# speedinghzl/DSRG

Hardware: NVIDIA H100
Metric: images/s, SRG + DenseCRF pass at 321x321x21 (higher is better)
Workload: dtype f32

## Files before the change

dsrg_b200/csrc/api.cu:

```cuda
#include <math.h>
#include <stdarg.h>
#include <stdlib.h>
#include <string.h>

#include <map>
#include <mutex>
#include <utility>
#include <new>
#include <vector>

#include "common.cuh"

namespace dsrg {

static thread_local char g_err[512] = "";

void set_error(const char *fmt, ...) {
    va_list ap;
    va_start(ap, fmt);
    vsnprintf(g_err, sizeof(g_err), fmt, ap);
    va_end(ap);
}

int device_alloc(Engine *e, void **p, size_t bytes) {
    if (bytes == 0) bytes = 16;
    cudaError_t err = cudaMalloc(p, bytes);
    if (err != cudaSuccess) {
        set_error("cudaMalloc(%zu bytes) failed: %s", bytes, cudaGetErrorString(err));
        *p = nullptr;
        return DSRG_E_NOMEM;
    }
    e->bytes += bytes;
    return DSRG_OK;
}

static void lattice_scales(Lattice &L) {
    const float inv_std_dev = (float)(sqrt(2.0 / 3.0) * (L.d + 1));
    for (int i = 0; i < L.d; i++)
        L.scale[i] = (float)(1.0 / sqrt((double)((i + 2) * (i + 1))) * (double)inv_std_dev);
}

static bool key_range_ok(const Lattice &L, int W, int H) {
    double fmax[5] = {(W - 1) / (double)L.sigma[0], (H - 1) / (double)L.sigma[1], 0, 0, 0};
    for (int i = 2; i < L.d; i++) fmax[i] = 255.0 / (double)L.sigma[i];
    double sum = 0, big = 0;
    for (int i = 0; i < L.d; i++) {
        double cf = fabs(fmax[i]) * L.scale[i];
        sum += cf;
        if ((i + 1) * cf > big) big = (i + 1) * cf;
    }
    const double bound = sum + big + 3.0 * (L.d + 1) + 2;
    const int bits = (L.d == 2) ? 16 : 12;
    return bound < (double)((1 << (bits - 1)) - 1) && isfinite(bound);
}

static void lattice_shape(Engine *e, Lattice &L) {
    L.N = e->N;
    L.P = (4 - (e->N % 4)) % 4;
    L.capv = (L.N + L.P) * (L.d + 1);
    L.cap = 2 * L.capv;
    L.rows_cap = (long long)e->maxB * (L.capv + 1);
    L.nbr_stride = L.shared ? (long long)L.capv + 1 : L.rows_cap;
}

static void engine_shape(Engine *e, int H, int W) {
    e->H = H;
    e->W = W;
    e->N = H * W;
    e->tiles_x = (W + kTileW - 1) / kTileW;
    e->tile_w = (W + e->tiles_x - 1) / e->tiles_x;
    e->tiles_y = (H + kTileH - 1) / kTileH;
    e->ntiles = e->tiles_x * e->tiles_y;
    lattice_shape(e, e->sp);
    lattice_shape(e, e->bi);
    e->sp_valid = false;
}

static int lattice_alloc(Engine *e, Lattice &L, int d, int shared) {
    L.d = d;
    L.shared = shared;
    L.nimg = shared ? 1 : e->maxB;
    lattice_shape(e, L);
    const size_t n = (size_t)L.nimg;
    int rc = 0;
    rc |= dalloc(e, &L.off, n * (d + 1) * L.N);
    rc |= dalloc(e, &L.bary, n * (d + 1) * L.N);
    rc |= dalloc(e, &L.norm, n * L.N);
    rc |= dalloc(e, &L.hkeys, n * L.cap);
    rc |= dalloc(e, &L.hval, n * L.cap);
    rc |= dalloc(e, &L.vslot, n * L.capv);
    rc |= dalloc(e, &L.vcount, n);
    rc |= dalloc(e, &L.aslot, n * L.capv);
    rc |= dalloc(e, &L.vkey, n * L.capv);
    const long long rn_words = renum_words(e->ntiles, d + 1);
    rc |= dalloc(e, &L.rn_words, n * rn_words);
    rc |= dalloc(e, &L.rn_chunk, n * (rn_words / kRenumChunk));
    rc |= dalloc(e, &L.rowbase, (size_t)e->maxB + 1);
    rc |= dalloc(e, &L.nbr, (size_t)(d + 1) * L.nbr_stride);
    L.maxloc = (d == 2) ? kMaxLocSp : kMaxLocHy;
    const size_t nt = n * e->ntiles;
    rc |= dalloc(e, &L.tl_nloc, nt);
    rc |= dalloc(e, &L.tl_hy, nt);
    L.entcap = (kTileThreads * (d + 1) + L.maxloc + 7) & ~7;
    rc |= dalloc(e, &L.tl_hdr, nt * L.maxloc);
    rc |= dalloc(e, &L.tl_pack, nt * L.entcap);
    rc |= dalloc(e, &L.tl_loc, n * (d + 1) * L.N);
    rc |= dalloc(e, &L.wn, n * (d + 1) * L.N);
    if (rc) return DSRG_E_NOMEM;
    if (cudaMemset(L.hkeys, 0xFF, sizeof(uint64_t) * n * L.cap) != cudaSuccess) return DSRG_E_CUDA;
    if (cudaMemset(L.tl_hy, 0, nt) != cudaSuccess) return DSRG_E_CUDA;
    if (cudaMemset(L.hval, 0xFF, sizeof(int32_t) * n * L.cap) != cudaSuccess) return DSRG_E_CUDA;
    if (cudaMemset(L.vkey, 0x7F, sizeof(int32_t) * n * L.capv) != cudaSuccess) return DSRG_E_CUDA;
    return DSRG_OK;
}

static void lattice_free(Lattice &L) {
    cudaFree(L.off);
    cudaFree(L.bary);
    cudaFree(L.norm);
    cudaFree(L.hkeys);
    cudaFree(L.hval);
    cudaFree(L.vslot);
    cudaFree(L.vcount);
    cudaFree(L.aslot);
    cudaFree(L.vkey);
    cudaFree(L.rn_words);
    cudaFree(L.rn_chunk);
    cudaFree(L.rowbase);
    cudaFree(L.nbr);
    cudaFree(L.tl_nloc);
    cudaFree(L.tl_hy);
    cudaFree(L.tl_hdr);
    cudaFree(L.tl_pack);
    cudaFree(L.tl_loc);
    cudaFree(L.wn);
}

int check_device_flag(Engine *e, cudaStream_t s) {
    int flag = 0;
    DSRG_CUDA_TRY(cudaMemcpyAsync(&flag, e->dev_err, sizeof(int), cudaMemcpyDeviceToHost, s));
    DSRG_CUDA_TRY(cudaStreamSynchronize(s));
    if (flag != 0) {
        cudaMemsetAsync(e->dev_err, 0, sizeof(int), s);
        set_error("lattice coordinates exceed the packed-key range (sigma too small for this image size)");
        return flag;
    }
    return DSRG_OK;
}

static int prepare_lattices(Engine *e, int B, const uint8_t *image, const dsrg_crf_params &p,
                            cudaStream_t s) {
    if (!(p.theta_gamma_x > 0 && p.theta_gamma_y > 0 && p.theta_alpha_x > 0 && p.theta_alpha_y > 0 &&
          p.theta_beta_r > 0 && p.theta_beta_g > 0 && p.theta_beta_b > 0) || p.n_iters < 0) {
        set_error("CRF parameters must be positive");
        return DSRG_E_INVALID;
    }
    if (!e->sp_valid || e->sp.sigma[0] != p.theta_gamma_x || e->sp.sigma[1] != p.theta_gamma_y) {
        e->sp.sigma[0] = p.theta_gamma_x;
        e->sp.sigma[1] = p.theta_gamma_y;
        if (!key_range_ok(e->sp, e->W, e->H)) {
            set_error("spatial sigma (%g,%g) too small for %dx%d: lattice keys exceed 16 bits",
                      p.theta_gamma_x, p.theta_gamma_y, e->W, e->H);
            return DSRG_E_KEYRANGE;
        }
        int rc = lattice_build(e, e->sp, B, nullptr, s);
        if (rc) return rc;
        e->sp_valid = true;
    }
    e->bi.sigma[0] = p.theta_alpha_x;
    e->bi.sigma[1] = p.theta_alpha_y;
    e->bi.sigma[2] = p.theta_beta_r;
    e->bi.sigma[3] = p.theta_beta_g;
    e->bi.sigma[4] = p.theta_beta_b;
    if (!key_range_ok(e->bi, e->W, e->H)) {
        set_error("bilateral sigmas too small for %dx%d: lattice keys exceed the 12-bit packed range",
                  e->W, e->H);
        return DSRG_E_KEYRANGE;
    }
    return lattice_build(e, e->bi, B, image, s);
}

int check_batch(Engine *e, int B) {
    if (!e) {
        set_error("engine is NULL");
        return DSRG_E_INVALID;
    }
    if (B < 1 || B > e->maxB) {
        set_error("batch %d outside [1, %d]", B, e->maxB);
        return DSRG_E_INVALID;
    }
    int cur = -1;
    if (cudaGetDevice(&cur) != cudaSuccess || cur != e->device) DSRG_CUDA_TRY(cudaSetDevice(e->device));
    return DSRG_OK;
}

static bool spatial_ready(const Engine *e, const dsrg_crf_params *p) {
    return p && e->sp_valid && e->sp.sigma[0] == p->theta_gamma_x && e->sp.sigma[1] == p->theta_gamma_y;
}

static int crf_pass_done(Engine *e, int B, int rc) {
    if (rc == DSRG_OK) {
        e->Qcur = e->Q0;
        e->last_crf_B = B;
    } else {
        e->last_crf_B = 0;
    }
    return rc;
}

static GraphKey pass_key(const Engine *e, int entry, int B, const dsrg_crf_params *p) {
    GraphKey k;
    k.add(entry).add(B).add(e->H).add(e->W);
    if (p) k.add(*p);
    return k;
}

static int crf_core(Engine *e, int B, const float *unary, int layout, bool clamp, float *unary_rw,
                    const uint8_t *image, const dsrg_crf_params *p, cudaStream_t s) {
    if (layout != DSRG_LAYOUT_NHWC && layout != DSRG_LAYOUT_NCHW) {
        set_error("bad layout %d", layout);
        return DSRG_E_INVALID;
    }
    int rc = prepare_lattices(e, B, image, *p, s);
    if (rc) return rc;
    return meanfield_run(e, B, unary, layout, clamp, unary_rw, *p, s);
}

int crf_core_batch_for_post(Engine *e, int B, const float *unary_hwc, const uint8_t *images,
                            const dsrg_crf_params *p, cudaStream_t s) {
    return crf_core(e, B, unary_hwc, DSRG_LAYOUT_NHWC, false, nullptr, images, p, s);
}

bool post_pass_needs_spatial(const Engine *e, const dsrg_crf_params *p) { return !spatial_ready(e, p); }
void post_pass_done(Engine *e, const dsrg_crf_params *p, int B, int rc) {
    if (rc == DSRG_OK && p) {
        e->sp.sigma[0] = p->theta_gamma_x;
        e->sp.sigma[1] = p->theta_gamma_y;
        e->sp_valid = true;
    }
    crf_pass_done(e, B, rc);
}

int ensure_staging(Engine *e) {
    if (e->st_unary) return DSRG_OK;
    const size_t n = (size_t)e->maxB * e->M * e->Ncap;
    int rc = 0;
    rc |= dalloc(e, &e->st_unary, n);
    rc |= dalloc(e, &e->st_out, n);
    rc |= dalloc(e, &e->st_cues, n);
    rc |= dalloc(e, &e->st_labels, (size_t)e->maxB * e->M);
    rc |= dalloc(e, &e->st_image, (size_t)e->maxB * e->Ncap * 3);
    rc |= dalloc(e, &e->st_lmap, (size_t)e->maxB * e->Ncap);
    rc |= dalloc(e, &e->st_sel, (size_t)e->M);
    return rc ? DSRG_E_NOMEM : DSRG_OK;
}

int grow_staging(Engine *e, void **buf, size_t *cap_bytes, size_t bytes) {
    if (bytes <= *cap_bytes) return DSRG_OK;
    cudaFree(*buf);
    *buf = nullptr;
    *cap_bytes = 0;
    if (int rc = device_alloc(e, buf, bytes)) return rc;
    *cap_bytes = bytes;
    return DSRG_OK;
}

static int no_engine() {
    set_error("engine is NULL");
    return DSRG_E_INVALID;
}

static int last_crf_held(const Engine *e, int B) {
    if (e->last_crf_B == B) return DSRG_OK;
    set_error("no mean-field result for a batch of %d is held by this engine (last: %d)", B, e->last_crf_B);
    return DSRG_E_STATE;
}

static bool layout_ok(int layout) { return layout == DSRG_LAYOUT_NHWC || layout == DSRG_LAYOUT_NCHW; }

}

using namespace dsrg;

extern "C" {

int dsrg_version(void) { return 109; }

const char *dsrg_last_error(void) { return g_err; }

int dsrg_device_count(void) {
    int n = 0;
    if (cudaGetDeviceCount(&n) != cudaSuccess) {
        cudaGetLastError();
        return 0;
    }
    return n;
}

int dsrg_current_device(void) {
    if (const char *ev = getenv("DSRG_B200_DEVICE")) return atoi(ev);
    int dev = -1;
    if (cudaGetDevice(&dev) != cudaSuccess) {
        cudaGetLastError();
        return -1;
    }
    return dev;
}

void *dsrg_host_alloc(size_t bytes) {
    void *p = nullptr;
    if (numa_host_alloc(&p, bytes ? bytes : 16, dsrg_current_device()) != cudaSuccess) {
        set_error("cudaHostAlloc(%zu) failed", bytes);
        cudaGetLastError();
        return nullptr;
    }
    return p;
}

void dsrg_host_free(void *p) {
    if (p) cudaFreeHost(p);
}

int dsrg_host_register(void *p, size_t bytes) {
    if (!p || !bytes) return DSRG_E_INVALID;
    if (cudaHostRegister(p, bytes, cudaHostRegisterDefault) != cudaSuccess) {
        cudaGetLastError();
        set_error("cudaHostRegister(%zu bytes) failed", bytes);
        return DSRG_E_CUDA;
    }
    return DSRG_OK;
}

int dsrg_host_unregister(void *p) {
    if (!p) return DSRG_E_INVALID;
    if (cudaHostUnregister(p) != cudaSuccess) {
        cudaGetLastError();
        return DSRG_E_CUDA;
    }
    return DSRG_OK;
}

void dsrg_crf_params_default(dsrg_crf_params *p, float scale_factor, float color_factor, int maxiter) {
    p->w1 = 10.0f;
    p->theta_alpha_x = p->theta_alpha_y = (float)(80.0 / (double)scale_factor);
    p->theta_beta_r = p->theta_beta_g = p->theta_beta_b = color_factor;
    p->w2 = 3.0f;
    p->theta_gamma_x = p->theta_gamma_y = (float)(3.0 / (double)scale_factor);
    p->n_iters = maxiter;
}

dsrg_engine *dsrg_engine_create(int device, int max_batch, int H, int W, int M) {
    if (max_batch < 1 || H < 1 || W < 1 || M < 1 || M > DSRG_MAX_LABELS_WIDE ||
        (long long)H * W > (1ll << 24)) {
        set_error("bad engine shape (max_batch=%d H=%d W=%d M=%d; M <= %d)", max_batch, H, W, M,
                  DSRG_MAX_LABELS_WIDE);
        return nullptr;
    }
    int ndev = 0;
    if (device < 0) device = dsrg_current_device();
    if (cudaGetDeviceCount(&ndev) != cudaSuccess || device < 0 || device >= ndev) {
        cudaGetLastError();
        set_error("no usable CUDA device %d (visible devices: %d): this library has no CPU fallback",
                  device, ndev);
        return nullptr;
    }
    cudaDeviceProp prop;
    Engine probe;
    probe.device = device;
    DeviceScope dev_scope(&probe);
    if (cudaGetDeviceProperties(&prop, device) != cudaSuccess) {
        set_error("cannot select device %d", device);
        return nullptr;
    }
    if (prop.major != 9 || prop.minor != 0) {
        set_error("device %d is sm_%d%d; this build contains sm_90a code only", device, prop.major,
                  prop.minor);
        return nullptr;
    }
    Engine *e = new (std::nothrow) Engine();
    if (!e) return nullptr;
    e->device = device;
    if (numa_wanted()) {
        e->numa_node = numa_node_of_device(device);
        numa_bind_thread(e->numa_node);
    }
    e->maxB = max_batch;
    e->M = M;
    e->MP = (M + 3) / 4 * 4;
    e->sm_count = prop.multiProcessorCount;
    e->sp.d = 2;
    e->sp.shared = 1;
    e->bi.d = 5;
    e->Hcap = H;
    e->Wcap = W;
    e->Ncap = H * W;
    engine_shape(e, H, W);
    int rc = 0;
    rc |= lattice_alloc(e, e->sp, 2, 1);
    rc |= lattice_alloc(e, e->bi, 5, 0);
    lattice_scales(e->sp);
    lattice_scales(e->bi);
    const size_t n = (size_t)max_batch * M * e->N;
    rc |= dalloc(e, &e->U, n);
    rc |= dalloc(e, &e->Q0, n);
    rc |= dalloc(e, &e->spA, (size_t)e->sp.rows_cap * e->MP);
    rc |= dalloc(e, &e->spB, (size_t)e->sp.rows_cap * e->MP);
    rc |= dalloc(e, &e->spC, (size_t)e->sp.rows_cap * e->MP);
    rc |= dalloc(e, &e->biC, (size_t)e->bi.rows_cap * e->MP);
    rc |= dalloc(e, &e->biA, (size_t)e->bi.rows_cap * e->MP);
    rc |= dalloc(e, &e->biB, (size_t)e->bi.rows_cap * e->MP);
    rc |= dalloc(e, &e->nvA, (size_t)e->bi.rows_cap);
    rc |= dalloc(e, &e->nvB, (size_t)e->bi.rows_cap);
    const size_t bn = (size_t)max_batch * e->N;
    rc |= dalloc(e, &e->lmap, bn);
    rc |= dalloc(e, &e->lflag, bn);
    rc |= dalloc(e, &e->parent, bn);
    rc |= dalloc(e, &e->hc, bn);
    rc |= dalloc(e, &e->loss_acc, (size_t)max_batch * 4);
    e->sec_wcap = e->Ncap < DSRG_GWRP_MAX_PLANE ? e->Ncap : DSRG_GWRP_MAX_PLANE;
    rc |= dalloc(e, &e->sec_rec, (size_t)max_batch * M);
    rc |= dalloc(e, &e->sec_img, (size_t)max_batch * 3);
    rc |= dalloc(e, &e->sec_part, (size_t)max_batch * kSecPlainChunks);
    rc |= dalloc(e, &e->sec_w, (size_t)2 * e->sec_wcap);
    rc |= dalloc(e, &e->dev_err, 1);
    rc |= dalloc(e, &e->hy_list, (size_t)max_batch * e->ntiles);
    rc |= dalloc(e, &e->hy_count, 1);
    if (!rc && cudaMemset(e->hy_count, 0, sizeof(int)) != cudaSuccess) rc = DSRG_E_CUDA;
    if (!rc && cudaMemset(e->dev_err, 0, sizeof(int)) != cudaSuccess) rc = DSRG_E_CUDA;
    if (!rc && cudaStreamCreateWithFlags(&e->own_stream, cudaStreamNonBlocking) != cudaSuccess) rc = DSRG_E_CUDA;
    if (!rc && cudaStreamCreateWithFlags(&e->in_stream, cudaStreamNonBlocking) != cudaSuccess) rc = DSRG_E_CUDA;
    if (!rc && cudaEventCreateWithFlags(&e->order_event, cudaEventDisableTiming) != cudaSuccess) rc = DSRG_E_CUDA;
    if (const char *ev = getenv("DSRG_B200_WIRE")) e->wire_compress = atoi(ev) != 0;
    if (const char *ev = getenv("DSRG_B200_GRAPHS")) e->use_graphs = atoi(ev) != 0;
    if (const char *ev = getenv("DSRG_B200_HOST_CHUNK")) e->host_chunk = atoi(ev) > 0 ? atoi(ev) : e->host_chunk;
    if (!rc && cudaStreamCreateWithFlags(&e->out_stream, cudaStreamNonBlocking) != cudaSuccess) rc = DSRG_E_CUDA;
    if (rc) {
        dsrg_engine_destroy((dsrg_engine *)e);
        return nullptr;
    }
    e->Qcur = e->Q0;
    return (dsrg_engine *)e;
}

void dsrg_engine_destroy(dsrg_engine *h) {
    Engine *e = (Engine *)h;
    if (!e) return;
    DeviceScope dev_scope(e);
    cudaDeviceSynchronize();
    graph_clear(e);
    lattice_free(e->sp);
    lattice_free(e->bi);
    void *ptrs[] = {e->U, e->Q0, e->spA, e->spB, e->spC, e->biA, e->biB, e->biC, e->nvA, e->nvB, e->lmap,
                    e->lflag, e->parent, e->hc, e->loss_acc, e->sec_rec, e->sec_img, e->sec_part, e->sec_w, e->dev_err,
                    e->hy_list, e->hy_count, e->st_unary, e->st_out, e->st_cues, e->st_labels, e->st_image, e->st_lmap, e->st_raw, e->st_idx,
                    e->st_prep, e->st_sel};
    for (void *p : ptrs) cudaFree(p);
    if (e->own_stream) cudaStreamDestroy(e->own_stream);
    if (e->in_stream) cudaStreamDestroy(e->in_stream);
    if (e->order_event) cudaEventDestroy(e->order_event);
    if (e->out_stream) cudaStreamDestroy(e->out_stream);
    for (auto ev : e->pipe_events) cudaEventDestroy(ev);
    wire_free(e);
    for (auto &r : e->prof_recs) {
        cudaEventDestroy(r.a);
        cudaEventDestroy(r.b);
    }
    for (auto ev : e->prof_pool) cudaEventDestroy(ev);
    delete e;
}

size_t dsrg_engine_device_bytes(const dsrg_engine *h) { return h ? ((const Engine *)h)->bytes : 0; }

static int set_size(Engine *e, int H, int W, bool wait) {
    if (!e) return no_engine();
    if (H < 1 || W < 1 || H > e->Hcap || W > e->Wcap) {
        set_error("size %dx%d outside the engine's capacity %dx%d", H, W, e->Hcap, e->Wcap);
        return DSRG_E_INVALID;
    }
    if (H == e->H && W == e->W) return DSRG_OK;
    if (wait) {
        DeviceScope dev_scope(e);
        DSRG_CUDA_TRY(cudaDeviceSynchronize());
    }
    engine_shape(e, H, W);
    e->last_crf_B = 0;
    return DSRG_OK;
}

int dsrg_engine_set_size(dsrg_engine *h, int H, int W) { return set_size((Engine *)h, H, W, true); }

int dsrg_engine_set_size_ordered(dsrg_engine *h, int H, int W) { return set_size((Engine *)h, H, W, false); }

int dsrg_engine_get_size(const dsrg_engine *h, int *H, int *W, int *Hcap, int *Wcap) {
    const Engine *e = (const Engine *)h;
    if (!e) return no_engine();
    if (H) *H = e->H;
    if (W) *W = e->W;
    if (Hcap) *Hcap = e->Hcap;
    if (Wcap) *Wcap = e->Wcap;
    return DSRG_OK;
}

long long dsrg_engine_take_launch_count(dsrg_engine *h) {
    Engine *e = (Engine *)h;
    if (!e) return 0;
    long long n = e->launches;
    e->launches = 0;
    return n;
}

static const char *kTagNames[T_COUNT] = {
    "lattice_insert", "lattice_misc", "lattice_norm", "mf_init", "mf_zero", "mf_blur_spatial",
    "mf_blur_bilateral", "mf_tile", "mf_export", "srg_label", "srg_merge", "srg_flag", "srg_emit",
    "seedloss", "wire_bits", "prepare_image", "postprocess", "annotation", "mf_tile_hybrid"};

int dsrg_profile_tag_count(void) { return T_COUNT; }

const char *dsrg_profile_tag_name(int tag) { return (tag >= 0 && tag < T_COUNT) ? kTagNames[tag] : ""; }

int dsrg_engine_set_host_chunk(dsrg_engine *h, int images) {
    Engine *e = (Engine *)h;
    if (!e) return no_engine();
    if (images < 0) return DSRG_E_INVALID;
    e->host_chunk = images;
    return DSRG_OK;
}

int dsrg_engine_set_graphs(dsrg_engine *h, int enable) {
    Engine *e = (Engine *)h;
    if (!e) return no_engine();
    e->use_graphs = enable != 0;
    if (!enable) {
        DeviceScope dev_scope(e);
        cudaDeviceSynchronize();
        graph_clear(e);
    }
    return DSRG_OK;
}

long long dsrg_engine_graph_replays(const dsrg_engine *h) { return h ? ((const Engine *)h)->graph_replays : 0; }
long long dsrg_engine_hybrid_tiles(dsrg_engine *h) {
    Engine *e = (Engine *)h;
    if (!e) return -1;
    DeviceScope dev_scope(e);
    int n = 0;
    if (cudaDeviceSynchronize() != cudaSuccess ||
        cudaMemcpy(&n, e->hy_count, sizeof(int), cudaMemcpyDeviceToHost) != cudaSuccess) {
        set_error("reading the hybrid-tile count failed: %s", cudaGetErrorString(cudaGetLastError()));
        return -1;
    }
    return n;
}

int dsrg_engine_profile(dsrg_engine *h, int enable) {
    Engine *e = (Engine *)h;
    if (!e) return no_engine();
    e->prof = enable != 0;
    return DSRG_OK;
}

int dsrg_engine_profile_read(dsrg_engine *h, float *ms_out, long long *count_out) {
    Engine *e = (Engine *)h;
    if (!e) return no_engine();
    if (!ms_out || !count_out) return DSRG_E_INVALID;
    DeviceScope dev_scope(e);
    DSRG_CUDA_TRY(cudaDeviceSynchronize());
    for (int t = 0; t < T_COUNT; t++) {
        ms_out[t] = 0.0f;
        count_out[t] = 0;
    }
    for (auto &r : e->prof_recs) {
        float ms = 0.0f;
        if (cudaEventElapsedTime(&ms, r.a, r.b) == cudaSuccess) {
            ms_out[r.tag] += ms;
            count_out[r.tag] += 1;
        }
        e->prof_pool.push_back(r.a);
        e->prof_pool.push_back(r.b);
    }
    e->prof_recs.clear();
    return DSRG_OK;
}

int dsrg_crf_batch_dev(dsrg_engine *h, int B, const float *unary, int unary_layout,
                       const uint8_t *image, const dsrg_crf_params *params, float *out,
                       int out_layout, void *stream) {
    const cudaStream_t s = (cudaStream_t)stream;
    return dev_call(h, B, s, unary && image && params && out && layout_ok(out_layout), [&](Engine *e) {
        GraphKey key = pass_key(e, 1, B, params);
        key.add(unary).add(unary_layout).add(image).add(out).add(out_layout);
        const bool rebuild = post_pass_needs_spatial(e, params);
        key.add(rebuild);
        if (rebuild) e->sp_valid = false;
        const int rc = run_pass(e, s, key, true, [&]() {
            int r = crf_core(e, B, unary, unary_layout, false, nullptr, image, params, s);
            if (r) return r;
            return meanfield_export(e, B, out, out_layout, s);
        });
        post_pass_done(e, params, B, rc);
        return rc;
    });
}

int dsrg_crf_map_batch_dev(dsrg_engine *h, int B, const float *unary, int unary_layout,
                           const uint8_t *image, const dsrg_crf_params *params, int32_t *labels_out,
                           void *stream) {
    const cudaStream_t s = (cudaStream_t)stream;
    return dev_call(h, B, s, unary && image && params && labels_out, [&](Engine *e) {
        GraphKey key = pass_key(e, 2, B, params);
        key.add(unary).add(unary_layout).add(image).add(labels_out);
        return crf_pass_done(e, B, run_pass(e, s, key, spatial_ready(e, params), [&]() {
            int r = crf_core(e, B, unary, unary_layout, false, nullptr, image, params, s);
            if (r) return r;
            return meanfield_export_map(e, B, labels_out, s);
        }));
    });
}

int dsrg_crf_batch_host(dsrg_engine *h, int B, const float *unary, int unary_layout,
                        const uint8_t *image, const dsrg_crf_params *params, float *out,
                        int out_layout) {
    return host_call(h, B, unary && image && params && out, true, [&](Engine *e, cudaStream_t s) {
        const size_t n = (size_t)B * e->M * e->N;
        DSRG_CUDA_TRY(cudaMemcpyAsync(e->st_unary, unary, n * sizeof(float), cudaMemcpyHostToDevice, s));
        DSRG_CUDA_TRY(cudaMemcpyAsync(e->st_image, image, (size_t)B * e->N * 3, cudaMemcpyHostToDevice, s));
        if (int rc = dsrg_crf_batch_dev(h, B, e->st_unary, unary_layout, e->st_image, params, e->st_out, out_layout, s))
            return rc;
        DSRG_CUDA_TRY(cudaMemcpyAsync(out, e->st_out, n * sizeof(float), cudaMemcpyDeviceToHost, s));
        return DSRG_OK;
    });
}

int dsrg_srg_batch_dev(dsrg_engine *h, int B, const float *labels, const float *probs,
                       const float *cues, double th1, double th2, int renorm, float *seeds_out,
                       int32_t *label_map_out, void *stream) {
    const cudaStream_t s = (cudaStream_t)stream;
    return dev_call(h, B, s, labels && probs && cues && seeds_out, [&](Engine *e) {
        if (e->M > 255) {
            set_error("SRG supports at most 255 classes");
            return DSRG_E_INVALID;
        }
        return srg_run(e, B, labels, probs, cues, th1, th2, renorm, seeds_out, label_map_out, s);
    });
}

}

namespace dsrg {
int dsrg_forward_core(Engine *e, int B, const float *labels, float *probs, const float *cues, const uint32_t *cue_bits,
                      const uint8_t *image, const dsrg_crf_params *params, double th1, double th2, float *seeds_out,
                      uint32_t *seed_bits, float *crf_out, cudaStream_t s) {
    GraphKey key = pass_key(e, 3, B, params);
    key.add(labels).add(probs).add(cues).add(cue_bits).add(image).add(th1).add(th2).add(seeds_out).add(seed_bits).add(crf_out);
    return crf_pass_done(e, B, run_pass(e, s, key, spatial_ready(e, params), [&]() {
        int r = crf_core(e, B, probs, DSRG_LAYOUT_NCHW, true, probs, image, params, s);
        if (r) return r;
        if (crf_out && (r = meanfield_export(e, B, crf_out, DSRG_LAYOUT_NCHW, s))) return r;
        return srg_run(e, B, labels, e->Qcur, cues, th1, th2, 1, seeds_out, nullptr, s, cue_bits, seed_bits);
    }));
}
}

extern "C" {

int dsrg_dsrg_forward_dev(dsrg_engine *h, int B, const float *labels, float *probs,
                          const float *cues, const uint8_t *image, const dsrg_crf_params *params,
                          double th1, double th2, float *seeds_out, float *crf_out, void *stream) {
    const cudaStream_t s = (cudaStream_t)stream;
    return dev_call(h, B, s, labels && probs && cues && image && params && seeds_out, [&](Engine *e) {
        return dsrg_forward_core(e, B, labels, probs, cues, nullptr, image, params, th1, th2, seeds_out, nullptr,
                                 crf_out, s);
    });
}

int dsrg_crflayer_forward_dev(dsrg_engine *h, int B, float *probs, const uint8_t *image,
                              const dsrg_crf_params *params, float *log_out, float *result,
                              void *stream) {
    const cudaStream_t s = (cudaStream_t)stream;
    return dev_call(h, B, s, probs && image && params && log_out, [&](Engine *e) {
        GraphKey key = pass_key(e, 4, B, params);
        key.add(probs).add(image).add(log_out).add(result);
        return crf_pass_done(e, B, run_pass(e, s, key, spatial_ready(e, params), [&]() {
            int r = crf_core(e, B, probs, DSRG_LAYOUT_NCHW, true, probs, image, params, s);
            if (r) return r;
            return meanfield_export_renorm(e, B, result, log_out, s);
        }));
    });
}

int dsrg_srg_last_crf_host(dsrg_engine *h, int B, const float *labels, const float *cues, double th1, double th2,
                           float *seeds_out) {
    return host_call(h, B, labels && cues && seeds_out, true, [&](Engine *e, cudaStream_t s) {
        const size_t n = (size_t)B * e->M * e->N;
        DSRG_CUDA_TRY(cudaMemcpyAsync(e->st_labels, labels, (size_t)B * e->M * sizeof(float), cudaMemcpyHostToDevice, s));
        DSRG_CUDA_TRY(cudaMemcpyAsync(e->st_cues, cues, n * sizeof(float), cudaMemcpyHostToDevice, s));
        if (int rc = srg_run(e, B, e->st_labels, e->Qcur, e->st_cues, th1, th2, 1, e->st_out, nullptr, s)) return rc;
        DSRG_CUDA_TRY(cudaMemcpyAsync(seeds_out, e->st_out, n * sizeof(float), cudaMemcpyDeviceToHost, s));
        return DSRG_OK;
    }, last_crf_held);
}

int dsrg_srg_last_crf_dev(dsrg_engine *h, const float *labels, const float *cues, int B, double th1, double th2,
                          float *seeds_out, void *stream) {
    const cudaStream_t s = (cudaStream_t)stream;
    return dev_call(h, B, s, labels && cues && seeds_out, [&](Engine *e) {
        if (int rc = last_crf_held(e, B)) return rc;
        return srg_run(e, B, labels, e->Qcur, cues, th1, th2, 1, seeds_out, nullptr, s);
    });
}

int dsrg_crf_last_marginals_host(dsrg_engine *h, int B, float *out, int out_layout) {
    return host_call(h, B, out && layout_ok(out_layout), false, [&](Engine *e, cudaStream_t s) {
        if (int rc = meanfield_export(e, B, e->st_out, out_layout, s)) return rc;
        DSRG_CUDA_TRY(cudaMemcpyAsync(out, e->st_out, (size_t)B * e->M * e->N * sizeof(float), cudaMemcpyDeviceToHost, s));
        return DSRG_OK;
    }, last_crf_held);
}

int dsrg_crflayer_forward_host(dsrg_engine *h, int B, float *probs, const uint8_t *image,
                               const dsrg_crf_params *params, float *log_out, float *result) {
    return host_call(h, B, probs && image && params && log_out, true, [&](Engine *e, cudaStream_t s) {
        const size_t n = (size_t)B * e->M * e->N;
        DSRG_CUDA_TRY(cudaMemcpyAsync(e->st_unary, probs, n * sizeof(float), cudaMemcpyHostToDevice, s));
        DSRG_CUDA_TRY(cudaMemcpyAsync(e->st_image, image, (size_t)B * e->N * 3, cudaMemcpyHostToDevice, s));
        if (int rc = dsrg_crflayer_forward_dev(h, B, e->st_unary, e->st_image, params, e->st_out,
                                               result ? e->st_cues : nullptr, s))
            return rc;
        DSRG_CUDA_TRY(cudaMemcpyAsync(log_out, e->st_out, n * sizeof(float), cudaMemcpyDeviceToHost, s));
        DSRG_CUDA_TRY(cudaMemcpyAsync(probs, e->st_unary, n * sizeof(float), cudaMemcpyDeviceToHost, s));
        if (result) DSRG_CUDA_TRY(cudaMemcpyAsync(result, e->st_cues, n * sizeof(float), cudaMemcpyDeviceToHost, s));
        return DSRG_OK;
    });
}

int dsrg_engine_lattice_sizes(dsrg_engine *h, int B, int *v_spatial, int *v_bilateral) {
    Engine *e = (Engine *)h;
    DeviceScope dev_scope(e);
    int rc = check_batch(e, B);
    if (rc) return rc;
    DSRG_CUDA_TRY(cudaDeviceSynchronize());
    if (v_spatial) DSRG_CUDA_TRY(cudaMemcpy(v_spatial, e->sp.vcount, sizeof(int), cudaMemcpyDeviceToHost));
    if (v_bilateral)
        DSRG_CUDA_TRY(cudaMemcpy(v_bilateral, e->bi.vcount, sizeof(int) * B, cudaMemcpyDeviceToHost));
    return DSRG_OK;
}

int dsrg_engine_lattice_tables(dsrg_engine *h, int which, int b, int *off_out, int *nbr_out) {
    Engine *e = (Engine *)h;
    DeviceScope dev_scope(e);
    int rc = check_entry(e, 1, e && (which == 0 || which == 1) && b >= 0 && b < e->maxB);
    if (rc) return rc;
    const Lattice &L = which == 0 ? e->sp : e->bi;
    const int sb = L.shared ? 0 : b;
    DSRG_CUDA_TRY(cudaDeviceSynchronize());
    int V = 0, base = 0;
    DSRG_CUDA_TRY(cudaMemcpy(&V, L.vcount + sb, sizeof(int), cudaMemcpyDeviceToHost));
    if (!L.shared) DSRG_CUDA_TRY(cudaMemcpy(&base, L.rowbase + b, sizeof(int), cudaMemcpyDeviceToHost));
    const int dp1 = L.d + 1;
    if (off_out)
        DSRG_CUDA_TRY(cudaMemcpy(off_out, L.off + (size_t)sb * dp1 * L.N, sizeof(int32_t) * dp1 * L.N,
                                 cudaMemcpyDeviceToHost));
    if (nbr_out) {
        for (int j = 0; j < dp1; j++) {
            int *dst = nbr_out + (size_t)j * (V + 1) * 2;
            DSRG_CUDA_TRY(cudaMemcpy(dst, L.nbr + (size_t)j * L.nbr_stride + base, sizeof(int2) * (V + 1),
                                     cudaMemcpyDeviceToHost));
            for (int k = 0; k < 2 * (V + 1); k++) dst[k] -= base;
        }
    }
    return DSRG_OK;
}

int dsrg_engine_copy_norm(dsrg_engine *h, int which, int B, float *norm_out) {
    Engine *e = (Engine *)h;
    DeviceScope dev_scope(e);
    int rc = check_entry(e, B, norm_out != nullptr);
    if (rc) return rc;
    DSRG_CUDA_TRY(cudaDeviceSynchronize());
    if (which == 0)
        DSRG_CUDA_TRY(cudaMemcpy(norm_out, e->sp.norm, sizeof(float) * e->N, cudaMemcpyDeviceToHost));
    else
        DSRG_CUDA_TRY(cudaMemcpy(norm_out, e->bi.norm, sizeof(float) * (size_t)B * e->N, cudaMemcpyDeviceToHost));
    return DSRG_OK;
}

struct dsrg_densecrf {
    int W, H, M;
    std::vector<float> unary;
    std::vector<unsigned char> image;
    dsrg_crf_params params;
    bool has_unary, has_pairwise;
};

static std::mutex g_pool_mu;
static std::map<std::pair<int, int>, Engine *> g_pool;

static Engine *pool_engine(int H, int W, int M) {
    const int dev = dsrg_current_device();
    Engine *&slot = g_pool[std::make_pair(dev, M)];
    Engine *e = slot;
    if (e && (H > e->Hcap || W > e->Wcap)) {
        H = H > e->Hcap ? H : e->Hcap;
        W = W > e->Wcap ? W : e->Wcap;
        dsrg_engine_destroy((dsrg_engine *)e);
        e = slot = nullptr;
    }
    if (!e) {
        const int Hc = (H + 63) / 64 * 64, Wc = (W + 63) / 64 * 64;
        e = slot = (Engine *)dsrg_engine_create(dev, 1, Hc, Wc, M);
        if (!e) return nullptr;
    }
    return e;
}

void dsrg_densecrf_release_engines(void) {
    std::lock_guard<std::mutex> lk(g_pool_mu);
    for (auto &kv : g_pool)
        if (kv.second) dsrg_engine_destroy((dsrg_engine *)kv.second);
    g_pool.clear();
}

dsrg_densecrf *dsrg_densecrf_create(int W, int H, int nlabels) {
    if (W < 1 || H < 1 || nlabels < 1 || nlabels > DSRG_MAX_LABELS_WIDE || (long long)H * W > (1ll << 24)) {
        set_error("bad shape (W=%d H=%d nlabels=%d; nlabels <= %d)", W, H, nlabels, DSRG_MAX_LABELS_WIDE);
        return nullptr;
    }
    if (dsrg_device_count() < 1) {
        set_error("no usable CUDA device: this library has no CPU fallback");
        return nullptr;
    }
    dsrg_densecrf *c = new (std::nothrow) dsrg_densecrf();
    if (!c) return nullptr;
    c->W = W;
    c->H = H;
    c->M = nlabels;
    c->has_unary = c->has_pairwise = false;
    return c;
}

void dsrg_densecrf_destroy(dsrg_densecrf *c) { delete c; }

int dsrg_densecrf_npixels(const dsrg_densecrf *c) { return c ? c->W * c->H : 0; }
int dsrg_densecrf_nlabels(const dsrg_densecrf *c) { return c ? c->M : 0; }

int dsrg_densecrf_set_unary_energy(dsrg_densecrf *c, const float *unary_costs) {
    if (!c || !unary_costs) {
        set_error("NULL pointer argument");
        return DSRG_E_INVALID;
    }
    const size_t n = (size_t)c->W * c->H * c->M;
    c->unary.resize(n);
    for (size_t i = 0; i < n; i++) c->unary[i] = -unary_costs[i];
    c->has_unary = true;
    return DSRG_OK;
}

int dsrg_densecrf_add_pairwise_energy(dsrg_densecrf *c, float w1, float theta_alpha_1,
                                      float theta_alpha_2, float theta_betta_1, float theta_betta_2,
                                      float theta_betta_3, float w2, float theta_gamma_1,
                                      float theta_gamma_2, const unsigned char *im) {
    if (!c || !im) {
        set_error("NULL pointer argument");
        return DSRG_E_INVALID;
    }
    if (c->has_pairwise) {
        set_error("add_pairwise_energy was already called on this object: only one Gaussian + bilateral pair is supported");
        return DSRG_E_STATE;
    }
    c->params.w1 = w1;
    c->params.theta_alpha_x = theta_alpha_1;
    c->params.theta_alpha_y = theta_alpha_2;
    c->params.theta_beta_r = theta_betta_1;
    c->params.theta_beta_g = theta_betta_2;
    c->params.theta_beta_b = theta_betta_3;
    c->params.w2 = w2;
    c->params.theta_gamma_x = theta_gamma_1;
    c->params.theta_gamma_y = theta_gamma_2;
    c->image.assign(im, im + (size_t)c->W * c->H * 3);
    c->has_pairwise = true;
    return DSRG_OK;
}

static int densecrf_engine(dsrg_densecrf *c, const void *out, Engine **e) {
    if (!c || !out) {
        set_error("bad argument (NULL pointer or value out of range)");
        return DSRG_E_INVALID;
    }
    *e = pool_engine(c->H, c->W, c->M);
    return *e ? DSRG_OK : DSRG_E_CUDA;
}

static int densecrf_run(dsrg_densecrf *c, int n_iters, Engine *e, cudaStream_t s) {
    int rc = dsrg_engine_set_size((dsrg_engine *)e, c->H, c->W);
    if (rc) return rc;
    if (!c->has_unary) c->unary.assign((size_t)c->W * c->H * c->M, 0.0f);
    c->params.n_iters = n_iters;
    DSRG_CUDA_TRY(cudaMemcpyAsync(e->st_unary, c->unary.data(), c->unary.size() * sizeof(float), cudaMemcpyHostToDevice, s));
    if (!c->has_pairwise) {
        dsrg_crf_params p0 = c->params;
        p0.n_iters = 0;
        return meanfield_run(e, 1, e->st_unary, DSRG_LAYOUT_NHWC, false, nullptr, p0, s);
    }
    DSRG_CUDA_TRY(cudaMemcpyAsync(e->st_image, c->image.data(), c->image.size(), cudaMemcpyHostToDevice, s));
    const bool rebuild = post_pass_needs_spatial(e, &c->params);
    GraphKey key = pass_key(e, 7, 1, &c->params);
    key.add(rebuild);
    if (rebuild) e->sp_valid = false;
    rc = run_pass(e, s, key, true, [&]() {
        return crf_core(e, 1, e->st_unary, DSRG_LAYOUT_NHWC, false, nullptr, e->st_image, &c->params, s);
    });
    post_pass_done(e, &c->params, 1, rc);
    return rc;
}

int dsrg_densecrf_inference(dsrg_densecrf *c, int n_iters, float *probs_out) {
    std::lock_guard<std::mutex> lk(g_pool_mu);
    Engine *eng = nullptr;
    if (int rc = densecrf_engine(c, probs_out, &eng)) return rc;
    return host_call((dsrg_engine *)eng, 1, true, true, [&](Engine *e, cudaStream_t s) {
        int rc = densecrf_run(c, n_iters, e, s);
        if (rc || (rc = meanfield_export(e, 1, e->st_out, DSRG_LAYOUT_NHWC, s))) return rc;
        DSRG_CUDA_TRY(cudaMemcpyAsync(probs_out, e->st_out, c->unary.size() * sizeof(float), cudaMemcpyDeviceToHost, s));
        return DSRG_OK;
    });
}

int dsrg_densecrf_map(dsrg_densecrf *c, int n_iters, int *labels) {
    std::lock_guard<std::mutex> lk(g_pool_mu);
    Engine *eng = nullptr;
    if (int rc = densecrf_engine(c, labels, &eng)) return rc;
    return host_call((dsrg_engine *)eng, 1, true, true, [&](Engine *e, cudaStream_t s) {
        int rc = densecrf_run(c, n_iters, e, s);
        if (rc || (rc = meanfield_export_map(e, 1, e->st_lmap, s))) return rc;
        DSRG_CUDA_TRY(cudaMemcpyAsync(labels, e->st_lmap, (size_t)c->W * c->H * sizeof(int), cudaMemcpyDeviceToHost, s));
        return DSRG_OK;
    });
}

}
```

dsrg_b200/csrc/common.cuh:

```cuda
#pragma once
#include <cuda_runtime.h>
#include <stdint.h>
#include <stdio.h>

#include <map>
#include <string>
#include <vector>

#include "../../include/dsrg_b200.h"

namespace dsrg {

constexpr int kThreads = 256;
constexpr uint64_t kEmptyKey = 0xFFFFFFFFFFFFFFFFull;
constexpr float kMinProb = 0.0001f;

void set_error(const char *fmt, ...);

#define DSRG_CUDA_TRY(expr)                                                              \
    do {                                                                                 \
        cudaError_t _e = (expr);                                                         \
        if (_e != cudaSuccess) {                                                         \
            dsrg::set_error("%s failed: %s (%s:%d)", #expr, cudaGetErrorString(_e),      \
                            __FILE__, __LINE__);                                         \
            return DSRG_E_CUDA;                                                          \
        }                                                                                \
    } while (0)

inline int cdiv(long long a, int b) { return (int)((a + b - 1) / b); }

struct Lattice {
    int d = 0;
    int shared = 0;
    int nimg = 0;
    int N = 0;
    int P = 0;
    int cap = 0;
    int capv = 0;
    long long rows_cap = 0;
    int32_t *off = nullptr;
    float *bary = nullptr;
    float *norm = nullptr;
    uint64_t *hkeys = nullptr;
    int32_t *hval = nullptr;
    int32_t *vslot = nullptr;
    int32_t *vcount = nullptr;
    int32_t *aslot = nullptr;
    int32_t *vkey = nullptr;
    uint2 *rn_words = nullptr;
    int32_t *rn_chunk = nullptr;
    int32_t *rowbase = nullptr;
    int2 *nbr = nullptr;
    long long nbr_stride = 0;
    int maxloc = 0;
    int32_t *tl_nloc = nullptr;
    uint8_t *tl_hy = nullptr;
    int2 *tl_hdr = nullptr;
    uint16_t *tl_pack = nullptr;
    int entcap = 0;
    uint16_t *tl_loc = nullptr;
    float *wn = nullptr;
    float scale[5] = {0, 0, 0, 0, 0};
    float sigma[5] = {0, 0, 0, 0, 0};
};

struct Engine;

enum KTag {
    T_LAT_INSERT = 0, T_LAT_MISC, T_LAT_NORM, T_MF_INIT, T_MF_ZERO, T_MF_BLUR_SP,
    T_MF_BLUR_BI, T_MF_TILE, T_MF_EXPORT, T_SRG_LABEL, T_SRG_MERGE, T_SRG_FLAG, T_SRG_EMIT,
    T_LOSS, T_WIRE, T_PREP, T_POST, T_ANNOT, T_MF_TILE_HY, T_COUNT
};

int lattice_build(Engine *e, Lattice &L, int B, const uint8_t *image_dev, cudaStream_t s);
constexpr int kNoKey = 0x7F7F7F7F;
constexpr int kRenumChunk = 4 * kThreads;
long long renum_words(int ntiles, int dp1);
constexpr int kTileW = 32, kTileH = 8;
constexpr int kTileThreads = kTileW * kTileH;
#ifndef DSRG_MAXLOC_BI
#define DSRG_MAXLOC_BI 192
#endif
#ifndef DSRG_TILE_CTAS
#define DSRG_TILE_CTAS 4
#endif
#ifndef DSRG_SPLAT_UNROLL
#define DSRG_SPLAT_UNROLL 8
#endif
#ifndef DSRG_ROW_PAD
#define DSRG_ROW_PAD 1
#endif
#ifndef DSRG_MAXLOC_SP
#define DSRG_MAXLOC_SP 128
#endif
#ifndef DSRG_MAXLOC_HY
#define DSRG_MAXLOC_HY 256
#endif
#ifndef DSRG_HY_CTAS
#define DSRG_HY_CTAS 3
#endif
constexpr int kMaxLocSp = DSRG_MAXLOC_SP, kMaxLocBi = DSRG_MAXLOC_BI, kMaxLocHy = DSRG_MAXLOC_HY;
static_assert(kMaxLocHy >= kMaxLocBi, "a hybrid tile holds at least what a plain one does");
constexpr int kSplatUnroll = DSRG_SPLAT_UNROLL;
constexpr int kLocRemote = 0xFFFF, kTileHybrid = 1 << 16;
static_assert(kTileThreads == 256, "the entry's low byte is the thread index");
constexpr int kEntRows = 9;
constexpr int kEntZero = kEntRows << 8;
__host__ __device__ constexpr int ent_r0(int dp1) { return dp1 == 3 ? 0 : 3; }
#ifndef DSRG_HY_MIN_TILES
#define DSRG_HY_MIN_TILES 8
#endif
#ifndef DSRG_HY_MIN_COVER
#define DSRG_HY_MIN_COVER 40
#endif
int tiles_build(Engine *e, Lattice &L, int nb, cudaStream_t s);
inline bool hybrid_tiles_on(const Engine *e, int B);
int meanfield_run(Engine *e, int B, const float *unary, int unary_layout, bool clamp_inplace,
                  float *unary_rw, const dsrg_crf_params &p, cudaStream_t s);
int meanfield_run_wide(Engine *e, int B, const float *unary, int unary_layout, bool clamp_inplace,
                       float *unary_rw, const dsrg_crf_params &p, cudaStream_t s);
int wide_weights(Engine *e, Lattice &L, int nb, cudaStream_t s);
int meanfield_export(Engine *e, int B, float *out, int layout, cudaStream_t s);
int meanfield_export_map(Engine *e, int B, int32_t *labels, cudaStream_t s);
int meanfield_export_renorm(Engine *e, int B, float *result_out, float *log_out, cudaStream_t s);
int srg_run(Engine *e, int B, const float *labels, const float *probs, const float *cues,
            double th1, double th2, int renorm, float *seeds_out, int32_t *label_map_out,
            cudaStream_t s, const uint32_t *cue_bits = nullptr, uint32_t *seed_bits = nullptr);
int dsrg_forward_core(Engine *e, int B, const float *labels, float *probs, const float *cues, const uint32_t *cue_bits,
                      const uint8_t *image, const dsrg_crf_params *params, double th1, double th2, float *seeds_out,
                      uint32_t *seed_bits, float *crf_out, cudaStream_t s);
bool post_pass_needs_spatial(const Engine *e, const dsrg_crf_params *p);
void post_pass_done(Engine *e, const dsrg_crf_params *p, int B, int rc);
constexpr int kSecPlainChunks = 16;

struct Engine {
    int device = 0;
    int numa_node = -1;
    int maxB = 0, H = 0, W = 0, M = 0, MP = 0, N = 0;
    int Hcap = 0, Wcap = 0, Ncap = 0;
    int sm_count = 132;
    size_t bytes = 0;
    long long launches = 0;

    Lattice sp, bi;
    bool sp_valid = false;

    float *U = nullptr, *Q0 = nullptr;
    float *Qcur = nullptr;
    int last_crf_B = 0;
    float *spA = nullptr, *spB = nullptr, *spC = nullptr, *biA = nullptr, *biB = nullptr, *biC = nullptr;
    int tiles_x = 0, tiles_y = 0, ntiles = 0;
    int tile_w = 32;
    int2 *hy_list = nullptr;
    int *hy_count = nullptr;
    float *nvA = nullptr, *nvB = nullptr;
    uint8_t *lmap = nullptr;
    uint8_t *lflag = nullptr;
    int32_t *parent = nullptr;
    uint8_t *hc = nullptr;
    double *loss_acc = nullptr;
    double2 *sec_rec = nullptr;
    double *sec_img = nullptr;
    double2 *sec_part = nullptr;
    double *sec_w = nullptr;
    int sec_wcap = 0;
    double sec_q[2] = {0, 0}, sec_z[2] = {0, 0};
    int sec_n[2] = {0, 0};
    std::vector<double> sec_w_host[2];
    float *st_unary = nullptr, *st_out = nullptr, *st_cues = nullptr, *st_labels = nullptr;
    uint8_t *st_image = nullptr;
    int32_t *st_sel = nullptr;
    float *st_raw = nullptr;
    size_t st_raw_cap = 0;
    int32_t *st_idx = nullptr;
    size_t st_idx_cap = 0;
    uint8_t *st_prep = nullptr;
    size_t st_prep_cap = 0;
    int32_t *st_lmap = nullptr;
    cudaStream_t own_stream = nullptr, in_stream = nullptr, out_stream = nullptr;
    cudaEvent_t order_event = nullptr;
    cudaStream_t last_stream = nullptr;
    bool last_stream_valid = false;
    std::vector<cudaEvent_t> pipe_events;
    int host_chunk = 0;
    uint32_t *d_cbits = nullptr, *d_sbits = nullptr, *d_mbits = nullptr;
    uint32_t *h_cbits = nullptr, *h_sbits = nullptr, *h_mbits = nullptr;
    int wire_compress = 1;
    int *dev_err = nullptr;
    struct GraphRec { cudaGraphExec_t exec = nullptr; long long launches = 0; unsigned long long last_use = 0; bool bad = false; };
    std::map<std::string, GraphRec> graphs;
    unsigned long long graph_clock = 0;
    int use_graphs = 1;
    long long graph_replays = 0;
    bool prof = false;
    struct ProfRec { int tag; cudaEvent_t a, b; };
    std::vector<ProfRec> prof_recs;
    std::vector<cudaEvent_t> prof_pool;
};

struct StreamScope {
    Engine *e;
    cudaStream_t s;
    bool live = false;
    StreamScope(Engine *e_, cudaStream_t s_) : e(e_), s(s_) {
        if (!e || !e->order_event) return;
        cudaStreamCaptureStatus st = cudaStreamCaptureStatusNone;
        if (cudaStreamIsCapturing(s, &st) != cudaSuccess) {
            cudaGetLastError();
            return;
        }
        if (st != cudaStreamCaptureStatusNone) return;
        live = true;
        if (e->last_stream_valid && e->last_stream != s && cudaStreamWaitEvent(s, e->order_event, 0) != cudaSuccess)
            cudaGetLastError();
    }
    ~StreamScope() {
        if (!live) return;
        if (cudaEventRecord(e->order_event, s) == cudaSuccess) {
            e->last_stream = s;
            e->last_stream_valid = true;
        } else {
            cudaGetLastError();
        }
    }
};

inline bool hybrid_tiles_on(const Engine *e, int B) {
    return e->MP <= DSRG_MAX_LABELS && (long long)e->ntiles * B >= 16LL * e->sm_count;
}

struct LaunchScope {
    Engine *e;
    cudaStream_t s;
    cudaEvent_t b = nullptr;
    LaunchScope(Engine *e_, int tag, cudaStream_t s_) : e(e_), s(s_) {
        e->launches++;
        if (e->prof) {
            cudaEvent_t a = take();
            b = take();
            cudaEventRecord(a, s);
            e->prof_recs.push_back({tag, a, b});
        }
    }
    ~LaunchScope() {
        if (b) cudaEventRecord(b, s);
    }
    cudaEvent_t take() {
        if (!e->prof_pool.empty()) {
            cudaEvent_t ev = e->prof_pool.back();
            e->prof_pool.pop_back();
            return ev;
        }
        cudaEvent_t ev;
        cudaEventCreate(&ev);
        return ev;
    }
};
#define DSRG_LAUNCH(e, tag, s, ...)          \
    do {                                     \
        dsrg::LaunchScope _ls((e), (tag), (s)); \
        __VA_ARGS__;                         \
    } while (0)


template <int NT, typename F>
__device__ __forceinline__ double numpy_sum_block(F get, int lo, int n_rt) {
    const int n = NT ? NT : n_rt;
    if (n < 8) {
        double res = 0.0;
#pragma unroll
        for (int i = 0; i < n; i++) res += get(lo + i);
        return res;
    }
    double r[8];
#pragma unroll
    for (int j = 0; j < 8; j++) r[j] = get(lo + j);
    int i = 8;
#pragma unroll
    for (; i < n - (n % 8); i += 8) {
#pragma unroll
        for (int j = 0; j < 8; j++) r[j] += get(lo + i + j);
    }
    double res = ((r[0] + r[1]) + (r[2] + r[3])) + ((r[4] + r[5]) + (r[6] + r[7]));
#pragma unroll
    for (; i < n; i++) res += get(lo + i);
    return res;
}
template <int NT, typename F>
__device__ __forceinline__ double numpy_sum(F get, int n_rt) {
    const int n = NT ? NT : n_rt;
    if (n <= 128) return numpy_sum_block<NT>(get, 0, n);
    int n2 = n / 2;
    n2 -= n2 % 8;
    const double lo = numpy_sum_block<0>(get, 0, n2);
    const int m = n - n2;
    if (m <= 128) return lo + numpy_sum_block<0>(get, n2, m);
    int m2 = m / 2;
    m2 -= m2 % 8;
    return lo + (numpy_sum_block<0>(get, n2, m2) + numpy_sum_block<0>(get, n2 + m2, m - m2));
}

struct DeviceScope {
    int prev = -1;
    bool switched = false;
    explicit DeviceScope(const Engine *e) : DeviceScope(e ? e->device : -1) {}
    explicit DeviceScope(int device) {
        if (device < 0) return;
        if (cudaGetDevice(&prev) != cudaSuccess) {
            cudaGetLastError();
            prev = -1;
        }
        if (prev != device) switched = cudaSetDevice(device) == cudaSuccess && prev >= 0;
    }
    ~DeviceScope() {
        if (switched) cudaSetDevice(prev);
    }
    DeviceScope(const DeviceScope &) = delete;
    DeviceScope &operator=(const DeviceScope &) = delete;
};

bool numa_wanted();
int numa_node_of_device(int device);
bool numa_bind_thread(int node);
bool numa_prefer_memory(int node);
cudaError_t numa_host_alloc(void **p, size_t bytes, int device);

struct GraphKey {
    std::string bytes;
    template <typename T>
    GraphKey &add(const T &v) {
        bytes.append(reinterpret_cast<const char *>(&v), sizeof(T));
        return *this;
    }
};
constexpr int kGraphRetry = 1;
int graph_begin(Engine *e, cudaStream_t s, const GraphKey &key, bool *captured);
int graph_end(Engine *e, cudaStream_t s, const GraphKey &key, bool captured, int body_rc, long long launches_before);
void graph_clear(Engine *e);
template <typename F>
inline int run_pass(Engine *e, cudaStream_t s, const GraphKey &key, bool allow_graph, F body) {
    if (!allow_graph) return body();
    bool cap = false;
    const long long l0 = e->launches;
    const int g = graph_begin(e, s, key, &cap);
    if (g != 0) return g < 0 ? g : DSRG_OK;
    int rc = body();
    if (!cap) return rc;
    rc = graph_end(e, s, key, cap, rc, l0);
    if (rc == kGraphRetry) {
        e->launches = l0;
        rc = body();
    }
    return rc;
}

int device_alloc(Engine *e, void **p, size_t bytes);
int check_batch(Engine *e, int B);
int ensure_staging(Engine *e);
int grow_staging(Engine *e, void **buf, size_t *cap_bytes, size_t bytes);
int check_device_flag(Engine *e, cudaStream_t s);
void wire_free(Engine *e);
template <typename T>
inline int dalloc(Engine *e, T **p, size_t count) {
    return device_alloc(e, (void **)p, count * sizeof(T));
}

inline int check_entry(Engine *e, int B, bool args_ok) {
    if (int rc = check_batch(e, B)) return rc;
    if (args_ok) return DSRG_OK;
    set_error("bad argument (NULL pointer or value out of range)");
    return DSRG_E_INVALID;
}

template <typename F>
inline int dev_call(dsrg_engine *h, int B, cudaStream_t s, bool args_ok, F body) {
    Engine *e = (Engine *)h;
    DeviceScope dev_scope(e);
    if (int rc = check_entry(e, B, args_ok)) return rc;
    StreamScope stream_scope(e, s);
    return body(e);
}

template <typename F>
inline int host_call(dsrg_engine *h, int B, bool args_ok, bool flag, F body,
                     int (*state)(const Engine *, int) = nullptr) {
    Engine *e = (Engine *)h;
    DeviceScope dev_scope(e);
    int rc = check_entry(e, B, args_ok);
    if (!rc && state) rc = state(e, B);
    if (rc || (rc = ensure_staging(e))) return rc;
    cudaStream_t s = e->own_stream;
    StreamScope stream_scope(e, s);
    if ((rc = body(e, s))) return rc;
    if (flag) return check_device_flag(e, s);
    DSRG_CUDA_TRY(cudaStreamSynchronize(s));
    return DSRG_OK;
}

}
```

dsrg_b200/csrc/meanfield.cu:

```cuda
#include "common.cuh"

namespace dsrg {

template <int MP>
__global__ void __launch_bounds__(kThreads)
k_mf_init(const float *unary, float *unary_rw, int layout, int clamp, float *U, float *Q, int M,
          int N) {
    const int b = blockIdx.y;
    const int i = blockIdx.x * blockDim.x + threadIdx.x;
    if (i >= N) return;
    float u[MP];
    float mx = -INFINITY;
#pragma unroll
    for (int k = 0; k < MP; k++) {
        if (k < M) {
            size_t at = (layout == DSRG_LAYOUT_NCHW) ? ((size_t)b * M + k) * N + i
                                                     : ((size_t)b * N + i) * M + k;
            float v = unary[at];
            if (clamp && v < kMinProb) {
                v = kMinProb;
                unary_rw[at] = v;
            }
            u[k] = v;
            mx = fmaxf(mx, v);
        }
    }
    float s = 0.0f;
#pragma unroll
    for (int k = 0; k < MP; k++)
        if (k < M) {
            U[((size_t)b * M + k) * N + i] = u[k];
            u[k] = expf(u[k] - mx);
            s += u[k];
        }
    if (Q) {
#pragma unroll
        for (int k = 0; k < MP; k++)
            if (k < M) Q[((size_t)b * M + k) * N + i] = u[k] / s;
    }
}

struct TileLat {
    const int32_t *off;
    const int32_t *rowbase;
    const int32_t *tl_nloc;
    const uint8_t *tl_hy;
    const int2 *tl_hdr;
    const uint16_t *tl_pack;
    const uint16_t *tl_loc;
    const float *wn;
    const float *val_in;
    float *val_out;
    int entcap;
    int shared;
};

enum { MODE_FIRST = 0, MODE_MID = 1, MODE_LAST = 2 };

__device__ __forceinline__ float exp_neg(float x) {
    const float kL2E = 1.4426950408889634f, kL2E_lo = 1.9259630e-8f, kLn2 = 0.6931471805599453f;
    const float t = x * kL2E;
    float r = fmaf(x, kL2E, -t);
    r = fmaf(x, kL2E_lo, r);
    float e;
    asm("ex2.approx.ftz.f32 %0, %1;" : "=f"(e) : "f"(t));
    return fmaf(e, r * kLn2, e);
}

__device__ __forceinline__ uint32_t smem_u32(const void *p) { return (uint32_t)__cvta_generic_to_shared(p); }
__device__ __forceinline__ void mbar_init(uint64_t *bar, uint32_t count) {
    asm volatile("mbarrier.init.shared::cta.b64 [%0], %1;" ::"r"(smem_u32(bar)), "r"(count) : "memory");
}
__device__ __forceinline__ void mbar_arrive_expect_tx(uint64_t *bar, uint32_t bytes) {
    asm volatile("mbarrier.arrive.expect_tx.shared::cta.b64 _, [%0], %1;" ::"r"(smem_u32(bar)), "r"(bytes) : "memory");
}
__device__ __forceinline__ bool mbar_try_wait(uint64_t *bar, uint32_t parity) {
    uint32_t ok;
    asm volatile(
        "{\n"
        ".reg .pred p;\n"
        "mbarrier.try_wait.parity.shared::cta.b64 p, [%1], %2;\n"
        "selp.u32 %0, 1, 0, p;\n"
        "}\n"
        : "=r"(ok)
        : "r"(smem_u32(bar)), "r"(parity)
        : "memory");
    return ok != 0;
}
__device__ __forceinline__ void mbar_wait(uint64_t *bar, uint32_t parity) {
    for (uint32_t spin = 0; !mbar_try_wait(bar, parity); ++spin)
        if (spin > (1u << 24)) __trap();
}
__device__ __forceinline__ void bulk_g2s(void *dst_smem, const void *src_gmem, uint32_t bytes, uint64_t *bar) {
    asm volatile("cp.async.bulk.shared::cluster.global.mbarrier::complete_tx::bytes [%0], [%1], %2, [%3];" ::"r"(
                     smem_u32(dst_smem)),
                 "l"(src_gmem), "r"(bytes), "r"(smem_u32(bar))
                 : "memory");
}

template <int MP>
struct TileRow {
    static constexpr int CH = MP / 4;
    static constexpr int CHP = CH + DSRG_ROW_PAD;
};

template <int MP, int MAXBI = kMaxLocBi>
struct TileStage {
    static constexpr int CH = MP / 4;
    static constexpr int CHP = TileRow<MP>::CHP;
    static constexpr int kRows = kMaxLocSp + MAXBI;
    static constexpr int kBufF4 = (kRows * CHP > kTileThreads * CHP) ? kRows * CHP : kTileThreads * CHP;
    static constexpr int kEntSp = (kTileThreads * 3 + kMaxLocSp + 7) & ~7, kEntBi = (kTileThreads * 6 + MAXBI + 7) & ~7;
    float4 buf[kBufF4];
    uint16_t ent[kEntSp + kEntBi];
    uint64_t bar;
};

template <int MP, int MAXBI = kMaxLocBi>
struct TileSmem {
    TileStage<MP, MAXBI> st;
    float wtab[kEntZero + 4];
};

__device__ __forceinline__ uint32_t ent_block_bytes(int2 last) {
    return ((uint32_t)((last.x & 0xffff) + (((last.x >> 16) + 1) & ~1)) * 2u + 15u) & ~15u;
}

__device__ __forceinline__ void tile_put_weights(float *wtab, const float *w_sp, const float *w_bi) {
#pragma unroll
    for (int r = 0; r < 3; r++) wtab[(ent_r0(3) + r) * kTileThreads + threadIdx.x] = w_sp[r];
#pragma unroll
    for (int r = 0; r < 6; r++) wtab[(ent_r0(6) + r) * kTileThreads + threadIdx.x] = w_bi[r];
}

template <int MP, int DP1>
__device__ __forceinline__ void tile_slice_smem(const float4 *vs, const uint16_t *loc, size_t stride,
                                                const float *w, float coef, float *t, bool tail1) {
    constexpr int CH = MP / 4, CHP = TileRow<MP>::CHP;
#pragma unroll
    for (int r = 0; r < DP1; r++) {
        const float4 *row = vs + (int)__ldg(loc + r * stride) * CHP;
        const float wr = coef * w[r];
#pragma unroll
        for (int c = 0; c < CH - 1; c++) {
            const float4 v = row[c];
            t[4 * c + 0] = fmaf(wr, v.x, t[4 * c + 0]);
            t[4 * c + 1] = fmaf(wr, v.y, t[4 * c + 1]);
            t[4 * c + 2] = fmaf(wr, v.z, t[4 * c + 2]);
            t[4 * c + 3] = fmaf(wr, v.w, t[4 * c + 3]);
        }
        constexpr int c = CH - 1;
        if (tail1) {
            const float v = reinterpret_cast<const float *>(row + c)[0];
            t[4 * c + 0] = fmaf(wr, v, t[4 * c + 0]);
        } else {
            const float4 v = row[c];
            t[4 * c + 0] = fmaf(wr, v.x, t[4 * c + 0]);
            t[4 * c + 1] = fmaf(wr, v.y, t[4 * c + 1]);
            t[4 * c + 2] = fmaf(wr, v.z, t[4 * c + 2]);
            t[4 * c + 3] = fmaf(wr, v.w, t[4 * c + 3]);
        }
    }
}

template <int MP, int DP1>
__device__ __forceinline__ void tile_slice_global(const float4 *vin, const int32_t *off, size_t stride,
                                                  int base, const float *w, float coef, float *t) {
    constexpr int CH = MP / 4;
#pragma unroll
    for (int r = 0; r < DP1; r++) {
        const float4 *row = vin + (size_t)(base + off[r * stride]) * CH;
        const float wr = coef * w[r];
#pragma unroll
        for (int c = 0; c < CH; c++) {
            const float4 v = row[c];
            t[4 * c + 0] = fmaf(wr, v.x, t[4 * c + 0]);
            t[4 * c + 1] = fmaf(wr, v.y, t[4 * c + 1]);
            t[4 * c + 2] = fmaf(wr, v.z, t[4 * c + 2]);
            t[4 * c + 3] = fmaf(wr, v.w, t[4 * c + 3]);
        }
    }
}

template <int MP, int DP1>
__device__ __forceinline__ unsigned tile_slice_mixed(const float4 *vs, const uint16_t *loc, const float4 *vin,
                                                     const int32_t *off, size_t stride, int base, const float *w,
                                                     float coef, float *t) {
    constexpr int CH = MP / 4, CHP = TileRow<MP>::CHP;
    unsigned remote = 0;
#pragma unroll
    for (int r = 0; r < DP1; r++) {
        const int l = (int)__ldg(loc + r * stride);
        const float wr = coef * w[r];
        if (l != kLocRemote) {
            const float4 *row = vs + l * CHP;
#pragma unroll
            for (int c = 0; c < CH; c++) {
                const float4 v = row[c];
                t[4 * c + 0] = fmaf(wr, v.x, t[4 * c + 0]);
                t[4 * c + 1] = fmaf(wr, v.y, t[4 * c + 1]);
                t[4 * c + 2] = fmaf(wr, v.z, t[4 * c + 2]);
                t[4 * c + 3] = fmaf(wr, v.w, t[4 * c + 3]);
            }
        } else {
            remote |= 1u << r;
            const float4 *row = vin + (size_t)(base + __ldg(off + r * stride)) * CH;
#pragma unroll
            for (int c = 0; c < CH; c++) {
                const float4 v = __ldg(row + c);
                t[4 * c + 0] = fmaf(wr, v.x, t[4 * c + 0]);
                t[4 * c + 1] = fmaf(wr, v.y, t[4 * c + 1]);
                t[4 * c + 2] = fmaf(wr, v.z, t[4 * c + 2]);
                t[4 * c + 3] = fmaf(wr, v.w, t[4 * c + 3]);
            }
        }
    }
    return remote;
}

template <int DP1>
__device__ __forceinline__ unsigned tile_remote_mask(const uint16_t *loc, size_t stride) {
    unsigned remote = 0;
#pragma unroll
    for (int r = 0; r < DP1; r++)
        if ((int)__ldg(loc + r * stride) == kLocRemote) remote |= 1u << r;
    return remote;
}

template <int MP>
__device__ __forceinline__ void tile_splat_csr(float4 *vout_sp, float4 *vout_bi, int n_sp, int n_bi,
                                               const int2 *hdr_sp, const int2 *hdr_bi, int base_sp, int base_bi,
                                               const uint16_t *ent_sp, const uint16_t *ent_bi, const float4 *qs,
                                               const float *wtab) {
    constexpr int CH = MP / 4, CHP = TileRow<MP>::CHP;
    constexpr int LPV = 8;
    constexpr int kPairUnroll = kSplatUnroll / 2 > 0 ? kSplatUnroll / 2 : 1;
    static_assert(CH <= LPV, "lane mapping");
    const int pairs_sp = n_sp * LPV, pairs = (n_sp + n_bi) * LPV;
    const int cq = threadIdx.x & (LPV - 1);
    if (cq >= CH) return;
    auto hdr_of = [&](int p) {
        const bool s = p < pairs_sp;
        return __ldg((s ? hdr_sp : hdr_bi) + (s ? p : p - pairs_sp) / LPV);
    };
    int2 hn = threadIdx.x < pairs ? hdr_of(threadIdx.x) : make_int2(0, 0);
    for (int p = threadIdx.x; p < pairs; p += kTileThreads) {
        const bool is_sp = p < pairs_sp;
        const int2 h = hn;
        if (p + kTileThreads < pairs) hn = hdr_of(p + kTileThreads);
        const uint32_t *ep = reinterpret_cast<const uint32_t *>((is_sp ? ent_sp : ent_bi) + (h.x & 0xffff));
        const int n2 = ((h.x >> 16) + 1) >> 1;
        const float4 *qb = qs + cq;
        float4 a = make_float4(0.f, 0.f, 0.f, 0.f);
#pragma unroll kPairUnroll
        for (int it = 0; it < n2; ++it) {
            const uint32_t en = ep[it];
            const uint32_t e0 = en & 0xffffu, e1 = en >> 16;
            const float w0 = wtab[e0], w1 = wtab[e1];
            const float4 q0 = qb[(e0 & 255u) * CHP];
            const float4 q1 = qb[(e1 & 255u) * CHP];
            a.x = fmaf(w0, q0.x, a.x);
            a.y = fmaf(w0, q0.y, a.y);
            a.z = fmaf(w0, q0.z, a.z);
            a.w = fmaf(w0, q0.w, a.w);
            a.x = fmaf(w1, q1.x, a.x);
            a.y = fmaf(w1, q1.y, a.y);
            a.z = fmaf(w1, q1.z, a.z);
            a.w = fmaf(w1, q1.w, a.w);
        }
        atomicAdd((is_sp ? vout_sp : vout_bi) + (size_t)((is_sp ? base_sp : base_bi) + h.y) * CH + cq, a);
    }
}

template <int MP, int DP1>
__device__ __forceinline__ void tile_splat_direct(float4 *vout, const int32_t *off, size_t stride,
                                                  int base, const float *w, const float *q) {
    constexpr int CH = MP / 4;
#pragma unroll
    for (int r = 0; r < DP1; r++) {
        float4 *row = vout + (size_t)(base + off[r * stride]) * CH;
#pragma unroll
        for (int c = 0; c < CH; c++)
            atomicAdd(row + c, make_float4(w[r] * q[4 * c], w[r] * q[4 * c + 1], w[r] * q[4 * c + 2],
                                           w[r] * q[4 * c + 3]));
    }
}

template <int MP, int DP1>
__device__ __forceinline__ void tile_splat_remote(float4 *vout, unsigned remote, const int32_t *off, size_t stride,
                                                  int base, const float *w, const float *q) {
    constexpr int CH = MP / 4;
#pragma unroll
    for (int r = 0; r < DP1; r++) {
        if (!(remote >> r & 1u)) continue;
        float4 *row = vout + (size_t)(base + __ldg(off + r * stride)) * CH;
#pragma unroll
        for (int c = 0; c < CH; c++)
            atomicAdd(row + c, make_float4(w[r] * q[4 * c], w[r] * q[4 * c + 1], w[r] * q[4 * c + 2],
                                           w[r] * q[4 * c + 3]));
    }
}

template <int MP, int MAXBI>
__device__ __forceinline__ const float4 *tile_park(TileSmem<MP, MAXBI> &smt, const float *t, const float *w_sp,
                                                   const float *w_bi) {
    constexpr int CH = MP / 4, CHP = TileStage<MP, MAXBI>::CHP;
    const int tid = threadIdx.x;
    __syncthreads();
    float4 *qs = smt.st.buf;
#pragma unroll
    for (int c = 0; c < CH; c++) qs[tid * CHP + c] = make_float4(t[4 * c], t[4 * c + 1], t[4 * c + 2], t[4 * c + 3]);
    tile_put_weights(smt.wtab, w_sp, w_bi);
    __syncthreads();
    return qs;
}

template <int MP, int MODE>
__device__ __forceinline__ void tile_update(float *t, int M, int N, float *__restrict__ Qout, int b, int pix, bool in) {
    float mx = -INFINITY;
#pragma unroll
    for (int k = 0; k < MP; k++)
        if (k < M) mx = fmaxf(mx, t[k]);
    float s = 0.0f;
#pragma unroll
    for (int k = 0; k < MP; k++) {
        t[k] = (k < M) ? exp_neg(t[k] - mx) : 0.0f;
        s += t[k];
    }
    const float inv = __frcp_rn(s);
#pragma unroll
    for (int k = 0; k < MP; k++) t[k] *= inv;
    if (MODE == MODE_LAST) {
        if (in) {
            float *Qb = Qout + (size_t)b * M * N + pix;
#pragma unroll
            for (int k = 0; k < MP; k++) {
                if (k < M) *Qb = t[k];
                Qb += N;
            }
        }
    }
}

template <int MP, int MODE>
__device__ __forceinline__ void tile_load_pixel(const float *U, float *U_rw, int clamp, int M, int N, int b, int pix,
                                                bool in, const float *wn_sp, const float *wn_bi, float *t,
                                                float *w_sp, float *w_bi) {
    {
        const size_t ub = (size_t)b * M * N + pix;
        const float *Ub = U + ub;
#pragma unroll
        for (int k = 0; k < MP; k++) {
            float v = 0.0f;
            if (in && k < M) v = (MODE == MODE_FIRST) ? *Ub : __ldg(Ub);
            if (MODE == MODE_FIRST) {
                if (clamp && in && k < M && v < kMinProb) {
                    v = kMinProb;
                    U_rw[ub + (size_t)k * N] = v;
                }
            }
            t[k] = v;
            Ub += N;
        }
    }
    {
        const float *p = wn_sp;
#pragma unroll
        for (int r = 0; r < 3; r++, p += N) w_sp[r] = in ? __ldg(p) : 0.0f;
        p = wn_bi;
#pragma unroll
        for (int r = 0; r < 6; r++, p += N) w_bi[r] = in ? __ldg(p) : 0.0f;
    }
}

template <int MP, int MODE>
__global__ void __launch_bounds__(kTileThreads, DSRG_TILE_CTAS)
k_mf_tile(const float *U, float *U_rw, int clamp, float *__restrict__ Qout, TileLat sp, TileLat bi, float c_sp,
          float c_bi, int M, int N, int W, int H, int tiles_x, int ntiles, int tile_w) {
    constexpr int kRowBytes = MP * 4;
    using SM = TileSmem<MP>;
    using ST = TileStage<MP>;
    extern __shared__ __align__(128) unsigned char smem_raw[];
    SM &smt = *reinterpret_cast<SM *>(smem_raw);
    ST &sm = smt.st;
    if (bi.tl_hy[(size_t)blockIdx.y * ntiles + blockIdx.x]) return;
    const int tile = blockIdx.x, b = blockIdx.y, tid = threadIdx.x;
    const int tx = tile % tiles_x, ty = tile / tiles_x;
    const int x = tx * tile_w + (tid & 31), y = ty * kTileH + (tid >> 5);
    const bool in = (tid & 31) < tile_w && x < W && y < H;
    const int pix = in ? y * W + x : 0;
    const int sb_sp = sp.shared ? 0 : b, sb_bi = bi.shared ? 0 : b;
    const size_t ti_sp = (size_t)sb_sp * ntiles + tile, ti_bi = (size_t)sb_bi * ntiles + tile;
    const int nl_sp = sp.tl_nloc[ti_sp], nl_bi = bi.tl_nloc[ti_bi];
    const bool fb_sp = nl_sp < 0, fb_bi = nl_bi < 0;
    const int n_sp = fb_sp ? 0 : nl_sp, n_bi = fb_bi ? 0 : nl_bi;
    const int base_sp = sp.rowbase[b], base_bi = bi.rowbase[b];
    constexpr int CHP = ST::CHP;
    float4 *vs_sp = sm.buf, *vs_bi = sm.buf + kMaxLocSp * CHP;
    const int2 *hdr_sp = sp.tl_hdr + ti_sp * kMaxLocSp, *hdr_bi = bi.tl_hdr + ti_bi * kMaxLocHy;
    uint16_t *ent_sp = sm.ent, *ent_bi = sm.ent + ST::kEntSp;
    const size_t strideN = (size_t)N;
    const size_t px_sp = (size_t)sb_sp * 3 * N + pix, px_bi = (size_t)sb_bi * 6 * N + pix;

    const int n_copies = (MODE != MODE_FIRST ? n_sp + n_bi : 0) + (MODE != MODE_LAST ? (n_sp > 0) + (n_bi > 0) : 0);
    if (tid == 0) {
        mbar_init(&sm.bar, n_copies > 0 ? n_copies : 1);
        smt.wtab[kEntZero] = 0.0f;
        asm volatile("fence.mbarrier_init.release.cluster;" ::: "memory");
    }
    __syncthreads();
    for (int i = tid; i < n_sp + n_bi; i += kTileThreads) {
        const bool is_sp = i < n_sp;
        const int lv = is_sp ? i : i - n_sp;
        const int2 h = __ldg((is_sp ? hdr_sp : hdr_bi) + lv);
        const int row = (is_sp ? base_sp : base_bi) + h.y;
        if (MODE != MODE_FIRST) {
            mbar_arrive_expect_tx(&sm.bar, kRowBytes);
            bulk_g2s((is_sp ? vs_sp : vs_bi) + lv * CHP, (is_sp ? sp.val_in : bi.val_in) + (size_t)row * MP,
                     kRowBytes, &sm.bar);
        }
        if (MODE != MODE_LAST && lv == (is_sp ? n_sp : n_bi) - 1) {
            const uint32_t bytes = ent_block_bytes(h);
            mbar_arrive_expect_tx(&sm.bar, bytes);
            bulk_g2s(is_sp ? ent_sp : ent_bi,
                     is_sp ? sp.tl_pack + ti_sp * sp.entcap : bi.tl_pack + ti_bi * bi.entcap, bytes, &sm.bar);
        }
    }
    if (n_copies == 0 && tid == 0) mbar_arrive_expect_tx(&sm.bar, 0);

    float t[MP], w_sp[3], w_bi[6];
    tile_load_pixel<MP, MODE>(U, U_rw, clamp, M, N, b, pix, in, sp.wn + px_sp, bi.wn + px_bi, t, w_sp, w_bi);
    mbar_wait(&sm.bar, 0);

#ifdef DSRG_NO_TAIL1
    const bool tail1 = false;
#else
    const bool tail1 = (M == MP - 3);
#endif
    if (MODE != MODE_FIRST && in) {
        if (!fb_sp)
            tile_slice_smem<MP, 3>(vs_sp, sp.tl_loc + px_sp, strideN, w_sp, c_sp, t, tail1);
        else
            tile_slice_global<MP, 3>(reinterpret_cast<const float4 *>(sp.val_in), sp.off + px_sp, strideN,
                                     base_sp, w_sp, c_sp, t);
        if (!fb_bi)
            tile_slice_smem<MP, 6>(vs_bi, bi.tl_loc + px_bi, strideN, w_bi, c_bi, t, tail1);
        else
            tile_slice_global<MP, 6>(reinterpret_cast<const float4 *>(bi.val_in), bi.off + px_bi, strideN,
                                     base_bi, w_bi, c_bi, t);
    }
    tile_update<MP, MODE>(t, M, N, Qout, b, pix, in);
    if (MODE == MODE_LAST) return;
    const float4 *qs = tile_park(smt, t, w_sp, w_bi);
    float4 *vout_sp = reinterpret_cast<float4 *>(sp.val_out), *vout_bi = reinterpret_cast<float4 *>(bi.val_out);
    if (fb_sp && in) tile_splat_direct<MP, 3>(vout_sp, sp.off + px_sp, strideN, base_sp, w_sp, t);
    if (fb_bi && in) tile_splat_direct<MP, 6>(vout_bi, bi.off + px_bi, strideN, base_bi, w_bi, t);
    tile_splat_csr<MP>(vout_sp, vout_bi, n_sp, n_bi, hdr_sp, hdr_bi, base_sp, base_bi, ent_sp, ent_bi, qs, smt.wtab);
}

template <int MP, int MODE>
__global__ void __launch_bounds__(kTileThreads, DSRG_HY_CTAS)
k_mf_tile_hy(const float *U, float *U_rw, int clamp, float *__restrict__ Qout, TileLat sp, TileLat bi, float c_sp,
             float c_bi, int M, int N, int W, int H, int tiles_x, int ntiles, int tile_w, const int2 *hy_list,
             const int *hy_count) {
    constexpr int kRowBytes = MP * 4;
    using ST = TileStage<MP, kMaxLocHy>;
    constexpr int CHP = ST::CHP;
    extern __shared__ __align__(128) unsigned char smem_raw[];
    TileSmem<MP, kMaxLocHy> &smt = *reinterpret_cast<TileSmem<MP, kMaxLocHy> *>(smem_raw);
    ST &sm = smt.st;
    const int tid = threadIdx.x;
    const int nhy = *hy_count;
    const size_t strideN = (size_t)N;
    float4 *vs_sp = sm.buf, *vs_bi = sm.buf + kMaxLocSp * CHP;
    uint16_t *ent_sp = sm.ent, *ent_bi = sm.ent + ST::kEntSp;
    if (tid == 0) smt.wtab[kEntZero] = 0.0f;
    float4 *vout_sp = reinterpret_cast<float4 *>(sp.val_out), *vout_bi = reinterpret_cast<float4 *>(bi.val_out);
    for (int item = blockIdx.x; item < nhy; item += gridDim.x) {
        const int2 bt = hy_list[item];
        const int tile = bt.x, b = bt.y;
        const int tx = tile % tiles_x, ty = tile / tiles_x;
        const int x = tx * tile_w + (tid & 31), y = ty * kTileH + (tid >> 5);
        const bool in = (tid & 31) < tile_w && x < W && y < H;
        const int pix = in ? y * W + x : 0;
        const int sb_sp = sp.shared ? 0 : b, sb_bi = bi.shared ? 0 : b;
        const size_t ti_sp = (size_t)sb_sp * ntiles + tile, ti_bi = (size_t)sb_bi * ntiles + tile;
        const int nl_sp = sp.tl_nloc[ti_sp], nl_bi = bi.tl_nloc[ti_bi];
        const bool hy_sp = nl_sp < 0, hy_bi = true;
        const int n_sp = nl_sp < 0 ? 0 : nl_sp, n_bi = nl_bi & 0xffff;
        const int base_sp = sp.rowbase[b], base_bi = bi.rowbase[b];
        const int2 *hdr_sp = sp.tl_hdr + ti_sp * kMaxLocSp, *hdr_bi = bi.tl_hdr + ti_bi * kMaxLocHy;
        const size_t px_sp = (size_t)sb_sp * 3 * N + pix, px_bi = (size_t)sb_bi * 6 * N + pix;

        const int n_copies = (MODE != MODE_FIRST ? n_sp + n_bi : 0) + (MODE != MODE_LAST ? (n_sp > 0) + (n_bi > 0) : 0);
        if (tid == 0) {
            mbar_init(&sm.bar, n_copies > 0 ? n_copies : 1);
            asm volatile("fence.mbarrier_init.release.cluster;" ::: "memory");
        }
        __syncthreads();
        asm volatile("fence.proxy.async.shared::cta;" ::: "memory");
        for (int i = tid; i < n_sp + n_bi; i += kTileThreads) {
            const bool is_sp = i < n_sp;
            const int lv = is_sp ? i : i - n_sp;
            const int2 h = __ldg((is_sp ? hdr_sp : hdr_bi) + lv);
            const int row = (is_sp ? base_sp : base_bi) + h.y;
            if (MODE != MODE_FIRST) {
                mbar_arrive_expect_tx(&sm.bar, kRowBytes);
                bulk_g2s((is_sp ? vs_sp : vs_bi) + lv * CHP, (is_sp ? sp.val_in : bi.val_in) + (size_t)row * MP,
                         kRowBytes, &sm.bar);
            }
            if (MODE != MODE_LAST && lv == (is_sp ? n_sp : n_bi) - 1) {
                const uint32_t bytes = ent_block_bytes(h);
                mbar_arrive_expect_tx(&sm.bar, bytes);
                bulk_g2s(is_sp ? ent_sp : ent_bi,
                         is_sp ? sp.tl_pack + ti_sp * sp.entcap : bi.tl_pack + ti_bi * bi.entcap, bytes, &sm.bar);
            }
        }
        if (n_copies == 0 && tid == 0) mbar_arrive_expect_tx(&sm.bar, 0);

        float t[MP], w_sp[3], w_bi[6];
        tile_load_pixel<MP, MODE>(U, U_rw, clamp, M, N, b, pix, in, sp.wn + px_sp, bi.wn + px_bi, t, w_sp, w_bi);
        mbar_wait(&sm.bar, 0);

        unsigned rm_sp = 0, rm_bi = 0;
        if (in) {
            if (MODE != MODE_FIRST) {
                rm_sp = tile_slice_mixed<MP, 3>(vs_sp, sp.tl_loc + px_sp, reinterpret_cast<const float4 *>(sp.val_in),
                                                sp.off + px_sp, strideN, base_sp, w_sp, c_sp, t);
                rm_bi = tile_slice_mixed<MP, 6>(vs_bi, bi.tl_loc + px_bi, reinterpret_cast<const float4 *>(bi.val_in),
                                                bi.off + px_bi, strideN, base_bi, w_bi, c_bi, t);
            } else {
                if (hy_sp) rm_sp = tile_remote_mask<3>(sp.tl_loc + px_sp, strideN);
                if (hy_bi) rm_bi = tile_remote_mask<6>(bi.tl_loc + px_bi, strideN);
            }
        }
        tile_update<MP, MODE>(t, M, N, Qout, b, pix, in);
        if (MODE != MODE_LAST) {
            if (rm_sp) tile_splat_remote<MP, 3>(vout_sp, rm_sp, sp.off + px_sp, strideN, base_sp, w_sp, t);
            if (rm_bi) tile_splat_remote<MP, 6>(vout_bi, rm_bi, bi.off + px_bi, strideN, base_bi, w_bi, t);
            const float4 *qs = tile_park(smt, t, w_sp, w_bi);
            tile_splat_csr<MP>(vout_sp, vout_bi, n_sp, n_bi, hdr_sp, hdr_bi, base_sp, base_bi, ent_sp, ent_bi, qs,
                               smt.wtab);
        }
        __syncthreads();
        if (tid == 0) asm volatile("mbarrier.inval.shared::cta.b64 [%0];" ::"r"(smem_u32(&sm.bar)) : "memory");
    }
}

template <int MP>
__global__ void __launch_bounds__(kThreads)
k_mf_zero(float4 *a, const int32_t *rowbase_a, float4 *c, const int32_t *rowbase_c, int B) {
    constexpr int CH = MP / 4;
    const long long na = (long long)rowbase_a[B] * CH, nc = (long long)rowbase_c[B] * CH;
    const float4 z = make_float4(0.f, 0.f, 0.f, 0.f);
    for (long long t = (long long)blockIdx.x * blockDim.x + threadIdx.x; t < na + nc;
         t += (long long)gridDim.x * blockDim.x) {
        if (t < na) a[t] = z; else c[t - na] = z;
    }
}

__device__ __forceinline__ float4 blur_step(float4 o, float4 a, float4 d) {
    float4 r;
    r.x = o.x + 0.5f * (a.x + d.x);
    r.y = o.y + 0.5f * (a.y + d.y);
    r.z = o.z + 0.5f * (a.z + d.z);
    r.w = o.w + 0.5f * (a.w + d.w);
    return r;
}

template <int N>
__device__ __forceinline__ void blur_expand(int *u, const int2 *na) {
#pragma unroll
    for (int i = N - 1; i >= 0; i--) {
        const int2 e = na[u[i]];
        u[3 * i] = u[i];
        u[3 * i + 1] = e.x;
        u[3 * i + 2] = e.y;
    }
}

template <int N>
__device__ __forceinline__ void blur_reduce(float4 *v) {
#pragma unroll
    for (int i = 0; i < N; i++) v[i] = blur_step(v[3 * i], v[3 * i + 1], v[3 * i + 2]);
}

#ifndef DSRG_BLUR_CACHED_ROWS
#define DSRG_BLUR_CACHED_ROWS 65536
#endif
constexpr int kBlurCachedRows = DSRG_BLUR_CACHED_ROWS;
__host__ __device__ constexpr int blur_cached_ctas(int mp) { return (mp == 4 || mp == 12 || mp == 28) ? 6 : 8; }
template <int MP, int AX, int CTAS>
__global__ void __launch_bounds__(kThreads, CTAS)
k_mf_blur(const float4 *in, float4 *out, const int2 *nbr, long long nbr_stride, const int32_t *rowbase, int B,
          int shared, float4 *zero, int gate) {
    constexpr int CH = MP / 4;
    constexpr int K = AX == 1 ? 3 : 9;
    static_assert(AX == 1 || AX == 2, "one or two axes per pass");
    const long long r0 = rowbase[0], rows = rowbase[B] - r0;
    if (gate && (rows > (long long)kBlurCachedRows * B) != (gate == 2)) return;
    const int rows_img = shared ? rowbase[1] : 0;
    const long long total = rows * CH;
    for (long long t = (long long)blockIdx.x * blockDim.x + threadIdx.x; t < total;
         t += (long long)gridDim.x * blockDim.x) {
        const long long lg = t / CH;
        const int c = (int)(t - lg * CH);
        const long long g = r0 + lg;
        const int img0 = shared ? ((int)g / rows_img) * rows_img : 0;
        int u[K];
        u[0] = (int)g - img0;
        blur_expand<1>(u, nbr + (AX - 1) * nbr_stride);
        if constexpr (AX == 2) blur_expand<3>(u, nbr);
        const float4 *src = in + (long long)img0 * CH + c;
        float4 v[K];
#pragma unroll
        for (int i = 0; i < K; i++) v[i] = src[(size_t)(unsigned)u[i] * CH];
        if constexpr (AX == 2) blur_reduce<3>(v);
        blur_reduce<1>(v);
        out[g * CH + c] = v[0];
        if (zero) zero[g * CH + c] = make_float4(0.f, 0.f, 0.f, 0.f);
    }
}

__global__ void __launch_bounds__(kThreads)
k_mf_export(const float *Q, float *out, int layout, int M, int N) {
    const int b = blockIdx.y;
    const int i = blockIdx.x * blockDim.x + threadIdx.x;
    if (i >= N) return;
    for (int k = 0; k < M; k++) {
        float v = Q[((size_t)b * M + k) * N + i];
        size_t at = (layout == DSRG_LAYOUT_NCHW) ? ((size_t)b * M + k) * N + i
                                                 : ((size_t)b * N + i) * M + k;
        out[at] = v;
    }
}

__global__ void __launch_bounds__(kThreads)
k_mf_export_map(const float *Q, int32_t *labels, int M, int N) {
    const int b = blockIdx.y;
    const int i = blockIdx.x * blockDim.x + threadIdx.x;
    if (i >= N) return;
    int m = 0;
    float best = Q[((size_t)b * M) * N + i];
    for (int k = 1; k < M; k++) {
        float v = Q[((size_t)b * M + k) * N + i];
        if (v > best) {
            best = v;
            m = k;
        }
    }
    labels[(size_t)b * N + i] = m;
}

__global__ void __launch_bounds__(kThreads)
k_mf_export_renorm(const float *Q, float *result_out, float *log_out, int M, int N) {
    const int b = blockIdx.y;
    const int i = blockIdx.x * blockDim.x + threadIdx.x;
    if (i >= N) return;
    auto clamped = [&](int k) {
        const double v = (double)Q[((size_t)b * M + k) * N + i];
        return v < 0.0001 ? 0.0001 : v;
    };
    const double s = numpy_sum<0>(clamped, M);
    for (int k = 0; k < M; k++) {
        size_t at = ((size_t)b * M + k) * N + i;
        double v = (double)Q[at];
        if (v < 0.0001) v = 0.0001;
        v = v / s;
        if (result_out) result_out[at] = (float)v;
        if (log_out) log_out[at] = (float)log(v);
    }
}

static TileLat make_tile_view(const Lattice &L, const float *val_in, float *val_out) {
    TileLat v;
    v.off = L.off;
    v.rowbase = L.rowbase;
    v.tl_nloc = L.tl_nloc;
    v.tl_hy = L.tl_hy;
    v.tl_hdr = L.tl_hdr;
    v.tl_pack = L.tl_pack;
    v.entcap = L.entcap;
    v.tl_loc = L.tl_loc;
    v.wn = L.wn;
    v.val_in = val_in;
    v.val_out = val_out;
    v.shared = L.shared;
    return v;
}

template <int MP>
static float *blur_all(Engine *e, const Lattice &L, float *buf, float *tmp, float *dead, int B, int tag, int grid,
                       cudaStream_t s) {
    float *src = buf, *dst = tmp;
    for (int j = 0; j <= L.d; j += 2) {
        const float4 *in = (const float4 *)src;
        const int2 *nbr = L.nbr + (size_t)j * L.nbr_stride;
        float4 *zero = j == 0 ? (float4 *)dead : nullptr;
        if (j == L.d) {
            DSRG_LAUNCH(e, tag, s, (k_mf_blur<MP, 1, 8><<<grid, kThreads, 0, s>>>(in, (float4 *)dst, nbr, L.nbr_stride,
                                                                                L.rowbase, B, L.shared, zero, 0)));
        } else if (L.shared) {
            DSRG_LAUNCH(e, tag, s, (k_mf_blur<MP, 2, 4><<<grid, kThreads, 0, s>>>(in, (float4 *)dst, nbr, L.nbr_stride,
                                                                                L.rowbase, B, L.shared, zero, 0)));
        } else if (L.capv <= kBlurCachedRows) {
            DSRG_LAUNCH(e, tag, s, (k_mf_blur<MP, 2, blur_cached_ctas(MP)><<<grid, kThreads, 0, s>>>(
                                       in, (float4 *)dst, nbr, L.nbr_stride, L.rowbase, B, L.shared, zero, 0)));
        } else {
            DSRG_LAUNCH(e, tag, s, (k_mf_blur<MP, 2, blur_cached_ctas(MP)><<<grid, kThreads, 0, s>>>(in, (float4 *)dst, nbr, L.nbr_stride,
                                                                                L.rowbase, B, L.shared, zero, 1)));
            DSRG_LAUNCH(e, tag, s, (k_mf_blur<MP, 2, 4><<<grid, kThreads, 0, s>>>(in, (float4 *)dst, nbr, L.nbr_stride,
                                                                                L.rowbase, B, L.shared, zero, 2)));
        }
        float *t = src;
        src = dst;
        dst = t;
    }
    return src;
}

template <int MP>
static int run_impl(Engine *e, int B, const float *unary, int layout, bool clamp, float *unary_rw,
                    const dsrg_crf_params &p, cudaStream_t s) {
    const int M = e->M, N = e->N;
    dim3 gp(cdiv(N, kThreads), B);
    const int T = p.n_iters;
    const bool direct = (layout == DSRG_LAYOUT_NCHW) && T > 0;
    const float *Usrc = direct ? unary : e->U;
    float *Urw = direct ? unary_rw : nullptr;
    const int tclamp = (direct && clamp) ? 1 : 0;
    if (!direct)
        DSRG_LAUNCH(e, T_MF_INIT, s,
                    k_mf_init<MP><<<gp, kThreads, 0, s>>>(unary, unary_rw, layout, clamp ? 1 : 0, e->U,
                                                          T == 0 ? e->Q0 : nullptr, M, N));
    e->Qcur = e->Q0;
    e->last_crf_B = B;
    if (T == 0) return DSRG_OK;
    const float alpha_sp = 1.0f / (1 + powf(2, -e->sp.d));
    const float alpha_bi = 1.0f / (1 + powf(2, -e->bi.d));
    const float c_sp = p.w2 * alpha_sp, c_bi = p.w1 * alpha_bi;
    const size_t smem = sizeof(TileSmem<MP>);
    const size_t smem_hy = sizeof(TileSmem<MP, kMaxLocHy>);
    static bool attr_done[64] = {false};
    const int dv = e->device & 63;
    if (!attr_done[dv]) {
        DSRG_CUDA_TRY(cudaFuncSetAttribute(k_mf_tile<MP, MODE_FIRST>, cudaFuncAttributeMaxDynamicSharedMemorySize, (int)smem));
        DSRG_CUDA_TRY(cudaFuncSetAttribute(k_mf_tile<MP, MODE_MID>, cudaFuncAttributeMaxDynamicSharedMemorySize, (int)smem));
        DSRG_CUDA_TRY(cudaFuncSetAttribute(k_mf_tile<MP, MODE_LAST>, cudaFuncAttributeMaxDynamicSharedMemorySize, (int)smem));
        DSRG_CUDA_TRY(cudaFuncSetAttribute(k_mf_tile_hy<MP, MODE_FIRST>, cudaFuncAttributeMaxDynamicSharedMemorySize, (int)smem_hy));
        DSRG_CUDA_TRY(cudaFuncSetAttribute(k_mf_tile_hy<MP, MODE_MID>, cudaFuncAttributeMaxDynamicSharedMemorySize, (int)smem_hy));
        DSRG_CUDA_TRY(cudaFuncSetAttribute(k_mf_tile_hy<MP, MODE_LAST>, cudaFuncAttributeMaxDynamicSharedMemorySize, (int)smem_hy));
        attr_done[dv] = true;
    }
#ifndef DSRG_BLUR_GRID
#define DSRG_BLUR_GRID 8
#endif
    const int bgrid = DSRG_BLUR_GRID * e->sm_count;
    const int hgrid = DSRG_HY_CTAS * e->sm_count;
    const bool hy_on = hybrid_tiles_on(e, B);
    const dim3 gt(e->ntiles, B);
    float *spX = e->spA, *spY = e->spB, *spZ = e->spC;
    float *biX = e->biA, *biY = e->biB, *biZ = e->biC;
    DSRG_LAUNCH(e, T_MF_ZERO, s,
                k_mf_zero<MP><<<bgrid, kThreads, 0, s>>>((float4 *)spY, e->sp.rowbase, (float4 *)biY, e->bi.rowbase, B));
#define DSRG_TILE_LAUNCH(MODEV, QOUT)                                                                                 \
    do {                                                                                                              \
        if (hy_on)                                                                                                    \
            DSRG_LAUNCH(e, T_MF_TILE_HY, s,                                                                           \
                        (k_mf_tile_hy<MP, MODEV><<<hgrid, kTileThreads, smem_hy, s>>>(                                \
                            Usrc, Urw, tclamp, QOUT, vsp, vbi, c_sp, c_bi, M, N, e->W, e->H, e->tiles_x, e->ntiles,   \
                            e->tile_w, e->hy_list, e->hy_count)));                                                    \
        DSRG_LAUNCH(e, T_MF_TILE, s,                                                                                  \
                    (k_mf_tile<MP, MODEV><<<gt, kTileThreads, smem, s>>>(Usrc, Urw, tclamp, QOUT, vsp, vbi, c_sp,     \
                                                                        c_bi, M, N, e->W, e->H, e->tiles_x,           \
                                                                        e->ntiles, e->tile_w)));                      \
    } while (0)
    for (int it = 0; it <= T; it++) {
        TileLat vsp = make_tile_view(e->sp, spX, spY), vbi = make_tile_view(e->bi, biX, biY);
        if (it == T) {
            DSRG_TILE_LAUNCH(MODE_LAST, e->Q0);
            break;
        }
        if (it == 0)
            DSRG_TILE_LAUNCH(MODE_FIRST, nullptr);
        else
            DSRG_TILE_LAUNCH(MODE_MID, nullptr);
        float *sp_res = blur_all<MP>(e, e->sp, spY, spZ, spX, B, T_MF_BLUR_SP, bgrid, s);
        float *bi_res = blur_all<MP>(e, e->bi, biY, biZ, biX, B, T_MF_BLUR_BI, bgrid, s);
        float *sp_other = (sp_res == spY) ? spZ : spY, *bi_other = (bi_res == biY) ? biZ : biY;
        float *nspY = spX, *nbiY = biX;
        spX = sp_res; spY = nspY; spZ = sp_other;
        biX = bi_res; biY = nbiY; biZ = bi_other;
    }
#undef DSRG_TILE_LAUNCH
    DSRG_CUDA_TRY(cudaGetLastError());
    return DSRG_OK;
}

int meanfield_run(Engine *e, int B, const float *unary, int unary_layout, bool clamp_inplace,
                  float *unary_rw, const dsrg_crf_params &p, cudaStream_t s) {
    if (e->MP > DSRG_MAX_LABELS) return meanfield_run_wide(e, B, unary, unary_layout, clamp_inplace, unary_rw, p, s);
    switch (e->MP) {
        case 4: return run_impl<4>(e, B, unary, unary_layout, clamp_inplace, unary_rw, p, s);
        case 8: return run_impl<8>(e, B, unary, unary_layout, clamp_inplace, unary_rw, p, s);
        case 12: return run_impl<12>(e, B, unary, unary_layout, clamp_inplace, unary_rw, p, s);
        case 16: return run_impl<16>(e, B, unary, unary_layout, clamp_inplace, unary_rw, p, s);
        case 20: return run_impl<20>(e, B, unary, unary_layout, clamp_inplace, unary_rw, p, s);
        case 24: return run_impl<24>(e, B, unary, unary_layout, clamp_inplace, unary_rw, p, s);
        case 28: return run_impl<28>(e, B, unary, unary_layout, clamp_inplace, unary_rw, p, s);
        case 32: return run_impl<32>(e, B, unary, unary_layout, clamp_inplace, unary_rw, p, s);
    }
    set_error("unsupported label count %d", e->M);
    return DSRG_E_INVALID;
}

int meanfield_export(Engine *e, int B, float *out, int layout, cudaStream_t s) {
    dim3 gp(cdiv(e->N, kThreads), B);
    DSRG_LAUNCH(e, T_MF_EXPORT, s, k_mf_export<<<gp, kThreads, 0, s>>>(e->Qcur, out, layout, e->M, e->N));
    DSRG_CUDA_TRY(cudaGetLastError());
    return DSRG_OK;
}

int meanfield_export_map(Engine *e, int B, int32_t *labels, cudaStream_t s) {
    dim3 gp(cdiv(e->N, kThreads), B);
    DSRG_LAUNCH(e, T_MF_EXPORT, s, k_mf_export_map<<<gp, kThreads, 0, s>>>(e->Qcur, labels, e->M, e->N));
    DSRG_CUDA_TRY(cudaGetLastError());
    return DSRG_OK;
}

int meanfield_export_renorm(Engine *e, int B, float *result_out, float *log_out, cudaStream_t s) {
    dim3 gp(cdiv(e->N, kThreads), B);
    DSRG_LAUNCH(e, T_MF_EXPORT, s, k_mf_export_renorm<<<gp, kThreads, 0, s>>>(e->Qcur, result_out, log_out, e->M, e->N));
    DSRG_CUDA_TRY(cudaGetLastError());
    return DSRG_OK;
}

}
```

dsrg_b200/csrc/srg.cu:

```cuda
#include "common.cuh"

namespace dsrg {

__device__ __forceinline__ int uf_find(const int32_t *parent, int x) {
    const volatile int32_t *vp = parent;
    int p = vp[x];
    while (p != x) {
        x = p;
        p = vp[x];
    }
    return x;
}

__device__ __forceinline__ void uf_union(int32_t *parent, int a, int b) {
    while (true) {
        a = uf_find(parent, a);
        b = uf_find(parent, b);
        if (a == b) return;
        if (a > b) {
            int t = a;
            a = b;
            b = t;
        }
        int old = atomicMin(parent + b, a);
        if (old == b) return;
        b = old;
    }
}

#ifndef DSRG_SRG_LABEL_CTAS
#define DSRG_SRG_LABEL_CTAS 1
#endif
template <bool CB>
__device__ __forceinline__ float cue_at(const float *cues_f, const uint32_t *cues_b, size_t img_base_f, size_t img_base_w,
                                        int c, int N, int i) {
    if (!CB) return __ldg(cues_f + img_base_f + (size_t)c * N + i);
    const size_t g = (size_t)c * N + i;
    return (__ldg(cues_b + img_base_w + (g >> 5)) >> (g & 31)) & 1u ? 1.0f : 0.0f;
}

template <int MT, bool CB>
__global__ void __launch_bounds__(kThreads, DSRG_SRG_LABEL_CTAS)
k_srg_label(const float *__restrict__ labels, const float *__restrict__ probs, const float *__restrict__ cues,
            const uint32_t *__restrict__ cue_bits, int wpi,
            double th1, double th2, int renorm, uint8_t *lmap, uint8_t *lflag, int32_t *parent, uint8_t *hc,
            int32_t *label_map_out, int Mrt, int N, int W) {
    const int M = MT ? MT : Mrt;
    const int b = blockIdx.y;
    const int i = blockIdx.x * blockDim.x + threadIdx.x;
    const bool in = i < N;
    int L = 0;
    if (in) {
        const float *lab = labels + (size_t)b * M;
        const float *pb = probs + (size_t)b * M * N + i;
        const size_t cbase_f = (size_t)b * M * N, cbase_w = (size_t)b * wpi;
        int cstar = -1;
        double best = 0.0, s = 0.0;
        float nseed = 0.0f;
        float cue_at_L = 0.0f;
        float cuv[MT ? MT : 1], pv[MT ? MT : 1];
        if (MT) {
#pragma unroll
            for (int c = 0; c < (MT ? MT : 1); c++) {
                cuv[c] = cue_at<CB>(cues, cue_bits, cbase_f, cbase_w, c, N, i);
                pv[c] = __ldg(pb + (size_t)c * N);
            }
        }
        constexpr bool kInline = MT >= 8 && MT <= 128;
        constexpr int kBody = MT - MT % 8;
        double r8[8] = {0, 0, 0, 0, 0, 0, 0, 0};
#pragma unroll
        for (int c = 0; c < M; c++) {
            const float cu = MT ? cuv[MT ? c : 0] : cue_at<CB>(cues, cue_bits, cbase_f, cbase_w, c, N, i);
            nseed += cu;
            if (cu > 0.0f) {
                L = c + 1;
                cue_at_L = cu;
            }
            double v = (double)(MT ? pv[MT ? c : 0] : pb[(size_t)c * N]);
            if (renorm && v < 0.0001) v = 0.0001;
            if (kInline && renorm) {
                if (c < 8) r8[c & 7] = v;
                else if (c < kBody) r8[c & 7] += v;
                else {
                    if (c == kBody) s = ((r8[0] + r8[1]) + (r8[2] + r8[3])) + ((r8[4] + r8[5]) + (r8[6] + r8[7]));
                    s += v;
                }
            }
            if (lab[c] == 1.0f && (cstar < 0 || v > best)) {
                best = v;
                cstar = c;
            }
        }
        if (renorm) {
            if (kInline) {
                if (MT == kBody) s = ((r8[0] + r8[1]) + (r8[2] + r8[3])) + ((r8[4] + r8[5]) + (r8[6] + r8[7]));
            } else {
                auto clamped = [&](int c) {
                    const double v = (double)(MT ? pv[MT ? c : 0] : pb[(size_t)c * N]);
                    return v < 0.0001 ? 0.0001 : v;
                };
                s = numpy_sum<MT>(clamped, M);
            }
            best = best / s;
        }
        if (cstar >= 0 && best > th2 && (cstar != 0 || best > th1)) {
            L = cstar + 1;
            cue_at_L = cue_at<CB>(cues, cue_bits, cbase_f, cbase_w, cstar, N, i);
        }
        uint8_t fl = 0;
        if (L > 0) {
            const bool present = lab[L - 1] == 1.0f;
            const bool own = cue_at_L == 1.0f;
            if (present && own) fl |= 1;
            if (!own && nseed == 1.0f) fl |= 2;
        }
        lmap[(size_t)b * N + i] = (uint8_t)L;
        lflag[(size_t)b * N + i] = fl;
        hc[(size_t)b * N + i] = 0;
        if (label_map_out) label_map_out[(size_t)b * N + i] = L;
    }
    const unsigned lane = threadIdx.x & 31;
    const int x = in ? i % W : 0;
    const int left = __shfl_up_sync(0xffffffffu, L, 1);
    const bool joins_left = in && lane > 0 && x > 0 && L > 0 && left == L;
    const unsigned brk = ~__ballot_sync(0xffffffffu, joins_left);
    if (in) {
        const unsigned below = brk & (0xffffffffu >> (31 - lane));
        const int head_lane = 31 - __clz(below);
        parent[(size_t)b * N + i] = i - ((int)lane - head_lane);
    }
}

__global__ void __launch_bounds__(kThreads)
k_srg_merge(const uint8_t *lmap, int32_t *parent, int N, int W) {
    const int b = blockIdx.y;
    const int i = blockIdx.x * blockDim.x + threadIdx.x;
    if (i >= N) return;
    const uint8_t *lm = lmap + (size_t)b * N;
    int32_t *par = parent + (size_t)b * N;
    const int L = lm[i];
    if (L == 0) return;
    const int x = i % W;
    if (x > 0 && (threadIdx.x & 31) == 0 && lm[i - 1] == L) uf_union(par, i, i - 1);
    if (i >= W) {
        const int n = i - W;
        if (lm[n] == L) {
            if (!(x > 0 && lm[i - 1] == L && lm[n - 1] == L)) uf_union(par, i, n);
        } else {
            if (x > 0 && lm[n - 1] == L) uf_union(par, i, n - 1);
            if (x < W - 1 && lm[n + 1] == L) uf_union(par, i, n + 1);
        }
    }
}

__global__ void __launch_bounds__(kThreads)
k_srg_flag(const uint8_t *lflag, int32_t *parent, uint8_t *hc, int N) {
    const int b = blockIdx.y;
    const int i = blockIdx.x * blockDim.x + threadIdx.x;
    if (i >= N) return;
    int32_t *par = parent + (size_t)b * N;
    const int root = uf_find(par, i);
    par[i] = root;
    if (lflag[(size_t)b * N + i] & 1) hc[(size_t)b * N + root] = 1;
}

template <int MT, bool CB, bool SB>
__global__ void __launch_bounds__(kThreads)
k_srg_emit(const float *__restrict__ cues, const uint32_t *__restrict__ cue_bits, int wpi, const uint8_t *lmap,
           const uint8_t *lflag, const int32_t *parent, const uint8_t *hc, float *__restrict__ seeds_out,
           uint32_t *__restrict__ seed_bits, int Mrt, int N) {
    const int M = MT ? MT : Mrt;
    const int b = blockIdx.y;
    const int i = blockIdx.x * blockDim.x + threadIdx.x;
    const bool in = i < N;
    if (!SB && !in) return;
    const size_t p = (size_t)b * N + (in ? i : 0);
    int grow_c = -1;
    if (in) {
        const int L = lmap[p];
        if (L > 0 && !(lflag[p] & 2)) {
            const int root = parent[p];
            if (hc[(size_t)b * N + root]) grow_c = L - 1;
        }
    }
    const size_t cbase_f = (size_t)b * M * N, cbase_w = (size_t)b * wpi;
    float *ob = seeds_out + (size_t)b * M * N + i;
    const int i0 = i & ~31;
    if (MT) {
        float v[MT ? MT : 1];
#pragma unroll
        for (int c = 0; c < (MT ? MT : 1); c++) v[c] = in ? cue_at<CB>(cues, cue_bits, cbase_f, cbase_w, c, N, i) : 0.0f;
#pragma unroll
        for (int c = 0; c < (MT ? MT : 1); c++) {
            const float o = (c == grow_c) ? 1.0f : v[c];
            if (!SB) {
                ob[(size_t)c * N] = o;
            } else {
                const unsigned m = __ballot_sync(0xffffffffu, in && o != 0.0f);
                if ((threadIdx.x & 31) == 0 && m) {
                    const size_t g0 = (size_t)c * N + i0;
                    const int sh = (int)(g0 & 31);
                    atomicOr(seed_bits + cbase_w + (g0 >> 5), m << sh);
                    if (sh && (m >> (32 - sh))) atomicOr(seed_bits + cbase_w + (g0 >> 5) + 1, m >> (32 - sh));
                }
            }
        }
    } else {
        for (int c = 0; c < M; c++) {
            const float o = (c == grow_c) ? 1.0f : (in ? cue_at<CB>(cues, cue_bits, cbase_f, cbase_w, c, N, i) : 0.0f);
            if (!SB) {
                ob[(size_t)c * N] = o;
            } else {
                const unsigned m = __ballot_sync(0xffffffffu, in && o != 0.0f);
                if ((threadIdx.x & 31) == 0 && m) {
                    const size_t g0 = (size_t)c * N + i0;
                    const int sh = (int)(g0 & 31);
                    atomicOr(seed_bits + cbase_w + (g0 >> 5), m << sh);
                    if (sh && (m >> (32 - sh))) atomicOr(seed_bits + cbase_w + (g0 >> 5) + 1, m >> (32 - sh));
                }
            }
        }
    }
}

int srg_run(Engine *e, int B, const float *labels, const float *probs, const float *cues,
            double th1, double th2, int renorm, float *seeds_out, int32_t *label_map_out,
            cudaStream_t s, const uint32_t *cue_bits, uint32_t *seed_bits) {
    const int N = e->N, M = e->M;
    if (seed_bits && !cue_bits) {
        set_error("SRG seed bits need cue bits");
        return DSRG_E_INVALID;
    }
    const int wpi = (int)(((size_t)M * N + 31) / 32);
    dim3 g(cdiv(N, kThreads), B);
#define DSRG_LABEL(MTV, CBV)                                                                                          \
    DSRG_LAUNCH(e, T_SRG_LABEL, s,                                                                                     \
                (k_srg_label<MTV, CBV><<<g, kThreads, 0, s>>>(labels, probs, cues, cue_bits, wpi, th1, th2, renorm, e->lmap, \
                                                              e->lflag, e->parent, e->hc, label_map_out, M, N, e->W)))
    if (M == 21) { if (cue_bits) DSRG_LABEL(21, true); else DSRG_LABEL(21, false); }
    else { if (cue_bits) DSRG_LABEL(0, true); else DSRG_LABEL(0, false); }
#undef DSRG_LABEL
    DSRG_LAUNCH(e, T_SRG_MERGE, s, k_srg_merge<<<g, kThreads, 0, s>>>(e->lmap, e->parent, N, e->W));
    DSRG_LAUNCH(e, T_SRG_FLAG, s, k_srg_flag<<<g, kThreads, 0, s>>>(e->lflag, e->parent, e->hc, N));
    if (seed_bits) DSRG_CUDA_TRY(cudaMemsetAsync(seed_bits, 0, (size_t)B * wpi * sizeof(uint32_t), s));
#define DSRG_EMIT(MTV, CBV, SBV)                                                                                       \
    DSRG_LAUNCH(e, T_SRG_EMIT, s,                                                                                      \
                (k_srg_emit<MTV, CBV, SBV><<<g, kThreads, 0, s>>>(cues, cue_bits, wpi, e->lmap, e->lflag, e->parent, e->hc, \
                                                                  seeds_out, seed_bits, M, N)))
#define DSRG_EMIT_MT(MTV)                                              \
    if (cue_bits && seed_bits) DSRG_EMIT(MTV, true, true);             \
    else if (cue_bits) DSRG_EMIT(MTV, true, false);                    \
    else DSRG_EMIT(MTV, false, false)
    if (M == 21) { DSRG_EMIT_MT(21); } else { DSRG_EMIT_MT(0); }
#undef DSRG_EMIT_MT
#undef DSRG_EMIT
    DSRG_CUDA_TRY(cudaGetLastError());
    return DSRG_OK;
}

}
```

Baseline: 3436.

## Fuse SRG labeling into the final mean-field tile kernel

Adds a MODE_LAST_SRG variant of the mean-field tile kernel that computes SRG winner and labels, seed copy and row-run union links directly from the in-register Q, removing the separate label pass that reread Q and cues. Hybrid tiles get a small follow-up kernel. The emit step becomes a grow kernel that starts from a copy of the cue bits and only ORs in grown pixels, instead of a memset plus full rewrite. The fused kernel uses a lower CTA-per-SM bound, which may reduce occupancy of the last iteration.

```diff
diff --git a/dsrg_b200/csrc/api.cu b/dsrg_b200/csrc/api.cu
--- a/dsrg_b200/csrc/api.cu
+++ b/dsrg_b200/csrc/api.cu
@@ -9,7 +9,7 @@
 #include <new>
 #include <vector>
 
-#include "common.cuh"
+#include "srg.cuh"
 
 namespace dsrg {
 
@@ -216,14 +216,14 @@
 }
 
 static int crf_core(Engine *e, int B, const float *unary, int layout, bool clamp, float *unary_rw,
-                    const uint8_t *image, const dsrg_crf_params *p, cudaStream_t s) {
+                    const uint8_t *image, const dsrg_crf_params *p, cudaStream_t s, const SrgArgs *srg = nullptr) {
     if (layout != DSRG_LAYOUT_NHWC && layout != DSRG_LAYOUT_NCHW) {
         set_error("bad layout %d", layout);
         return DSRG_E_INVALID;
     }
     int rc = prepare_lattices(e, B, image, *p, s);
     if (rc) return rc;
-    return meanfield_run(e, B, unary, layout, clamp, unary_rw, *p, s);
+    return meanfield_run(e, B, unary, layout, clamp, unary_rw, *p, s, srg);
 }
 
 int crf_core_batch_for_post(Engine *e, int B, const float *unary_hwc, const uint8_t *images,
@@ -650,13 +650,18 @@
 int dsrg_forward_core(Engine *e, int B, const float *labels, float *probs, const float *cues, const uint32_t *cue_bits,
                       const uint8_t *image, const dsrg_crf_params *params, double th1, double th2, float *seeds_out,
                       uint32_t *seed_bits, float *crf_out, cudaStream_t s) {
+    if (seed_bits && !cue_bits) {
+        set_error("SRG seed bits need cue bits");
+        return DSRG_E_INVALID;
+    }
     GraphKey key = pass_key(e, 3, B, params);
     key.add(labels).add(probs).add(cues).add(cue_bits).add(image).add(th1).add(th2).add(seeds_out).add(seed_bits).add(crf_out);
+    const SrgArgs srg = srg_args(e, labels, cues, cue_bits, seeds_out, seed_bits, th1, th2);
     return crf_pass_done(e, B, run_pass(e, s, key, spatial_ready(e, params), [&]() {
-        int r = crf_core(e, B, probs, DSRG_LAYOUT_NCHW, true, probs, image, params, s);
+        int r = crf_core(e, B, probs, DSRG_LAYOUT_NCHW, true, probs, image, params, s, &srg);
         if (r) return r;
         if (crf_out && (r = meanfield_export(e, B, crf_out, DSRG_LAYOUT_NCHW, s))) return r;
-        return srg_run(e, B, labels, e->Qcur, cues, th1, th2, 1, seeds_out, nullptr, s, cue_bits, seed_bits);
+        return DSRG_OK;
     }));
 }
 }
diff --git a/dsrg_b200/csrc/common.cuh b/dsrg_b200/csrc/common.cuh
--- a/dsrg_b200/csrc/common.cuh
+++ b/dsrg_b200/csrc/common.cuh
@@ -84,6 +84,9 @@
 #ifndef DSRG_TILE_CTAS
 #define DSRG_TILE_CTAS 4
 #endif
+#ifndef DSRG_TILE_SRG_CTAS
+#define DSRG_TILE_SRG_CTAS 2
+#endif
 #ifndef DSRG_SPLAT_UNROLL
 #define DSRG_SPLAT_UNROLL 8
 #endif
@@ -115,8 +118,9 @@
 #endif
 int tiles_build(Engine *e, Lattice &L, int nb, cudaStream_t s);
 inline bool hybrid_tiles_on(const Engine *e, int B);
+struct SrgArgs;
 int meanfield_run(Engine *e, int B, const float *unary, int unary_layout, bool clamp_inplace,
-                  float *unary_rw, const dsrg_crf_params &p, cudaStream_t s);
+                  float *unary_rw, const dsrg_crf_params &p, cudaStream_t s, const SrgArgs *srg = nullptr);
 int meanfield_run_wide(Engine *e, int B, const float *unary, int unary_layout, bool clamp_inplace,
                        float *unary_rw, const dsrg_crf_params &p, cudaStream_t s);
 int wide_weights(Engine *e, Lattice &L, int nb, cudaStream_t s);
diff --git a/dsrg_b200/csrc/meanfield.cu b/dsrg_b200/csrc/meanfield.cu
--- a/dsrg_b200/csrc/meanfield.cu
+++ b/dsrg_b200/csrc/meanfield.cu
@@ -1,4 +1,4 @@
-#include "common.cuh"
+#include "srg.cuh"
 
 namespace dsrg {
 
@@ -55,7 +55,7 @@
     int shared;
 };
 
-enum { MODE_FIRST = 0, MODE_MID = 1, MODE_LAST = 2 };
+enum { MODE_FIRST = 0, MODE_MID = 1, MODE_LAST = 2, MODE_LAST_SRG = 3 };
 
 __device__ __forceinline__ float exp_neg(float x) {
     const float kL2E = 1.4426950408889634f, kL2E_lo = 1.9259630e-8f, kLn2 = 0.6931471805599453f;
@@ -330,7 +330,7 @@
     const float inv = __frcp_rn(s);
 #pragma unroll
     for (int k = 0; k < MP; k++) t[k] *= inv;
-    if (MODE == MODE_LAST) {
+    if (MODE >= MODE_LAST) {
         if (in) {
             float *Qb = Qout + (size_t)b * M * N + pix;
 #pragma unroll
@@ -340,6 +340,35 @@
             }
         }
     }
+}
+
+template <int MP>
+__device__ __forceinline__ void tile_srg(const SrgArgs &a, const float *t, int M, int N, int b, int pix, int x,
+                                         bool in) {
+    int L = 0;
+    if (in) {
+        const float *lab = a.labels + (size_t)b * M;
+        int cstar;
+        const double best = srg_winner<MP>([&](int c) { return t[c]; }, lab, M, 1, cstar);
+        const size_t cbase_f = (size_t)b * M * N, cbase_w = (size_t)b * a.wpi;
+        auto cue_mem = [&](int c) { return cue_at(a.cues, a.cue_bits, cbase_f, cbase_w, c, N, pix); };
+        float cuv[MP];
+#pragma unroll
+        for (int c = 0; c < MP; c++) cuv[c] = c < M ? cue_mem(c) : 0.0f;
+        if (float *sd = a.seed_copy()) {
+            sd += cbase_f + pix;
+#pragma unroll
+            for (int c = 0; c < MP; c++)
+                if (c < M) sd[(size_t)c * N] = cuv[c];
+        }
+        uint8_t fl;
+        L = srg_label<MP>([&](int c) { return cuv[c]; }, cue_mem, lab, M, cstar, best, a.th1, a.th2, fl);
+        const size_t p = (size_t)b * N + pix;
+        a.lmap[p] = (uint8_t)L;
+        a.lflag[p] = fl;
+        a.hc[p] = 0;
+    }
+    srg_link_runs(L, in, x, pix, a.parent + (size_t)b * N);
 }
 
 template <int MP, int MODE>
@@ -374,9 +403,9 @@
 }
 
 template <int MP, int MODE>
-__global__ void __launch_bounds__(kTileThreads, DSRG_TILE_CTAS)
+__global__ void __launch_bounds__(kTileThreads, MODE == MODE_LAST_SRG ? DSRG_TILE_SRG_CTAS : DSRG_TILE_CTAS)
 k_mf_tile(const float *U, float *U_rw, int clamp, float *__restrict__ Qout, TileLat sp, TileLat bi, float c_sp,
-          float c_bi, int M, int N, int W, int H, int tiles_x, int ntiles, int tile_w) {
+          float c_bi, int M, int N, int W, int H, int tiles_x, int ntiles, int tile_w, SrgArgs srg) {
     constexpr int kRowBytes = MP * 4;
     using SM = TileSmem<MP>;
     using ST = TileStage<MP>;
@@ -402,7 +431,7 @@
     const size_t strideN = (size_t)N;
     const size_t px_sp = (size_t)sb_sp * 3 * N + pix, px_bi = (size_t)sb_bi * 6 * N + pix;
 
-    const int n_copies = (MODE != MODE_FIRST ? n_sp + n_bi : 0) + (MODE != MODE_LAST ? (n_sp > 0) + (n_bi > 0) : 0);
+    const int n_copies = (MODE != MODE_FIRST ? n_sp + n_bi : 0) + (MODE < MODE_LAST ? (n_sp > 0) + (n_bi > 0) : 0);
     if (tid == 0) {
         mbar_init(&sm.bar, n_copies > 0 ? n_copies : 1);
         smt.wtab[kEntZero] = 0.0f;
@@ -419,7 +448,7 @@
             bulk_g2s((is_sp ? vs_sp : vs_bi) + lv * CHP, (is_sp ? sp.val_in : bi.val_in) + (size_t)row * MP,
                      kRowBytes, &sm.bar);
         }
-        if (MODE != MODE_LAST && lv == (is_sp ? n_sp : n_bi) - 1) {
+        if (MODE < MODE_LAST && lv == (is_sp ? n_sp : n_bi) - 1) {
             const uint32_t bytes = ent_block_bytes(h);
             mbar_arrive_expect_tx(&sm.bar, bytes);
             bulk_g2s(is_sp ? ent_sp : ent_bi,
@@ -450,7 +479,10 @@
                                      base_bi, w_bi, c_bi, t);
     }
     tile_update<MP, MODE>(t, M, N, Qout, b, pix, in);
-    if (MODE == MODE_LAST) return;
+    if (MODE >= MODE_LAST) {
+        if (MODE == MODE_LAST_SRG) tile_srg<MP>(srg, t, M, N, b, pix, x, in);
+        return;
+    }
     const float4 *qs = tile_park(smt, t, w_sp, w_bi);
     float4 *vout_sp = reinterpret_cast<float4 *>(sp.val_out), *vout_bi = reinterpret_cast<float4 *>(bi.val_out);
     if (fb_sp && in) tile_splat_direct<MP, 3>(vout_sp, sp.off + px_sp, strideN, base_sp, w_sp, t);
@@ -548,6 +580,25 @@
 }
 
 template <int MP>
+__global__ void __launch_bounds__(kTileThreads)
+k_mf_srg_hy(const float *__restrict__ Q, SrgArgs srg, int M, int N, int W, int H, int tiles_x, int tile_w,
+            const int2 *hy_list, const int *hy_count) {
+    if ((int)blockIdx.x >= *hy_count) return;
+    const int tid = threadIdx.x;
+    const int2 bt = hy_list[blockIdx.x];
+    const int tile = bt.x, b = bt.y;
+    const int tx = tile % tiles_x, ty = tile / tiles_x;
+    const int x = tx * tile_w + (tid & 31), y = ty * kTileH + (tid >> 5);
+    const bool in = (tid & 31) < tile_w && x < W && y < H;
+    const int pix = in ? y * W + x : 0;
+    float t[MP];
+    const float *Qb = Q + (size_t)b * M * N + pix;
+#pragma unroll
+    for (int k = 0; k < MP; k++) t[k] = (in && k < M) ? __ldg(Qb + (size_t)k * N) : 0.0f;
+    tile_srg<MP>(srg, t, M, N, b, pix, x, in);
+}
+
+template <int MP>
 __global__ void __launch_bounds__(kThreads)
 k_mf_zero(float4 *a, const int32_t *rowbase_a, float4 *c, const int32_t *rowbase_c, int B) {
     constexpr int CH = MP / 4;
@@ -721,7 +772,7 @@
 
 template <int MP>
 static int run_impl(Engine *e, int B, const float *unary, int layout, bool clamp, float *unary_rw,
-                    const dsrg_crf_params &p, cudaStream_t s) {
+                    const dsrg_crf_params &p, const SrgArgs *srg, cudaStream_t s) {
     const int M = e->M, N = e->N;
     dim3 gp(cdiv(N, kThreads), B);
     const int T = p.n_iters;
@@ -747,6 +798,7 @@
         DSRG_CUDA_TRY(cudaFuncSetAttribute(k_mf_tile<MP, MODE_FIRST>, cudaFuncAttributeMaxDynamicSharedMemorySize, (int)smem));
         DSRG_CUDA_TRY(cudaFuncSetAttribute(k_mf_tile<MP, MODE_MID>, cudaFuncAttributeMaxDynamicSharedMemorySize, (int)smem));
         DSRG_CUDA_TRY(cudaFuncSetAttribute(k_mf_tile<MP, MODE_LAST>, cudaFuncAttributeMaxDynamicSharedMemorySize, (int)smem));
+        DSRG_CUDA_TRY(cudaFuncSetAttribute(k_mf_tile<MP, MODE_LAST_SRG>, cudaFuncAttributeMaxDynamicSharedMemorySize, (int)smem));
         DSRG_CUDA_TRY(cudaFuncSetAttribute(k_mf_tile_hy<MP, MODE_FIRST>, cudaFuncAttributeMaxDynamicSharedMemorySize, (int)smem_hy));
         DSRG_CUDA_TRY(cudaFuncSetAttribute(k_mf_tile_hy<MP, MODE_MID>, cudaFuncAttributeMaxDynamicSharedMemorySize, (int)smem_hy));
         DSRG_CUDA_TRY(cudaFuncSetAttribute(k_mf_tile_hy<MP, MODE_LAST>, cudaFuncAttributeMaxDynamicSharedMemorySize, (int)smem_hy));
@@ -759,6 +811,7 @@
     const int hgrid = DSRG_HY_CTAS * e->sm_count;
     const bool hy_on = hybrid_tiles_on(e, B);
     const dim3 gt(e->ntiles, B);
+    const SrgArgs sa = srg ? *srg : SrgArgs{};
     float *spX = e->spA, *spY = e->spB, *spZ = e->spC;
     float *biX = e->biA, *biY = e->biB, *biZ = e->biC;
     DSRG_LAUNCH(e, T_MF_ZERO, s,
@@ -767,18 +820,27 @@
     do {                                                                                                              \
         if (hy_on)                                                                                                    \
             DSRG_LAUNCH(e, T_MF_TILE_HY, s,                                                                           \
-                        (k_mf_tile_hy<MP, MODEV><<<hgrid, kTileThreads, smem_hy, s>>>(                                \
+                        (k_mf_tile_hy<MP, MODEV == MODE_LAST_SRG ? MODE_LAST : MODEV><<<hgrid, kTileThreads, smem_hy, s>>>(                                \
                             Usrc, Urw, tclamp, QOUT, vsp, vbi, c_sp, c_bi, M, N, e->W, e->H, e->tiles_x, e->ntiles,   \
                             e->tile_w, e->hy_list, e->hy_count)));                                                    \
         DSRG_LAUNCH(e, T_MF_TILE, s,                                                                                  \
                     (k_mf_tile<MP, MODEV><<<gt, kTileThreads, smem, s>>>(Usrc, Urw, tclamp, QOUT, vsp, vbi, c_sp,     \
                                                                         c_bi, M, N, e->W, e->H, e->tiles_x,           \
-                                                                        e->ntiles, e->tile_w)));                      \
+                                                                        e->ntiles, e->tile_w, sa)));                  \
     } while (0)
     for (int it = 0; it <= T; it++) {
         TileLat vsp = make_tile_view(e->sp, spX, spY), vbi = make_tile_view(e->bi, biX, biY);
         if (it == T) {
-            DSRG_TILE_LAUNCH(MODE_LAST, e->Q0);
+            if (!srg) {
+                DSRG_TILE_LAUNCH(MODE_LAST, e->Q0);
+                break;
+            }
+            DSRG_TILE_LAUNCH(MODE_LAST_SRG, e->Q0);
+            if (hy_on)
+                DSRG_LAUNCH(e, T_SRG_LABEL, s,
+                            (k_mf_srg_hy<MP><<<e->ntiles * B, kTileThreads, 0, s>>>(e->Q0, sa, M, N, e->W, e->H, e->tiles_x,
+                                                                           e->tile_w, e->hy_list, e->hy_count)));
+            if (int rc = srg_finish(e, B, sa, e->tile_w, s)) return rc;
             break;
         }
         if (it == 0)
@@ -798,17 +860,23 @@
 }
 
 int meanfield_run(Engine *e, int B, const float *unary, int unary_layout, bool clamp_inplace,
-                  float *unary_rw, const dsrg_crf_params &p, cudaStream_t s) {
+                  float *unary_rw, const dsrg_crf_params &p, cudaStream_t s, const SrgArgs *srg) {
+    if (srg && (e->MP > DSRG_MAX_LABELS || p.n_iters == 0)) {
+        int rc = meanfield_run(e, B, unary, unary_layout, clamp_inplace, unary_rw, p, s, nullptr);
+        if (rc) return rc;
+        return srg_run(e, B, srg->labels, e->Qcur, srg->cues, srg->th1, srg->th2, 1, srg->seeds, nullptr, s,
+                       srg->cue_bits, srg->seed_bits);
+    }
     if (e->MP > DSRG_MAX_LABELS) return meanfield_run_wide(e, B, unary, unary_layout, clamp_inplace, unary_rw, p, s);
     switch (e->MP) {
-        case 4: return run_impl<4>(e, B, unary, unary_layout, clamp_inplace, unary_rw, p, s);
-        case 8: return run_impl<8>(e, B, unary, unary_layout, clamp_inplace, unary_rw, p, s);
-        case 12: return run_impl<12>(e, B, unary, unary_layout, clamp_inplace, unary_rw, p, s);
-        case 16: return run_impl<16>(e, B, unary, unary_layout, clamp_inplace, unary_rw, p, s);
-        case 20: return run_impl<20>(e, B, unary, unary_layout, clamp_inplace, unary_rw, p, s);
-        case 24: return run_impl<24>(e, B, unary, unary_layout, clamp_inplace, unary_rw, p, s);
-        case 28: return run_impl<28>(e, B, unary, unary_layout, clamp_inplace, unary_rw, p, s);
-        case 32: return run_impl<32>(e, B, unary, unary_layout, clamp_inplace, unary_rw, p, s);
+        case 4: return run_impl<4>(e, B, unary, unary_layout, clamp_inplace, unary_rw, p, srg, s);
+        case 8: return run_impl<8>(e, B, unary, unary_layout, clamp_inplace, unary_rw, p, srg, s);
+        case 12: return run_impl<12>(e, B, unary, unary_layout, clamp_inplace, unary_rw, p, srg, s);
+        case 16: return run_impl<16>(e, B, unary, unary_layout, clamp_inplace, unary_rw, p, srg, s);
+        case 20: return run_impl<20>(e, B, unary, unary_layout, clamp_inplace, unary_rw, p, srg, s);
+        case 24: return run_impl<24>(e, B, unary, unary_layout, clamp_inplace, unary_rw, p, srg, s);
+        case 28: return run_impl<28>(e, B, unary, unary_layout, clamp_inplace, unary_rw, p, srg, s);
+        case 32: return run_impl<32>(e, B, unary, unary_layout, clamp_inplace, unary_rw, p, srg, s);
     }
     set_error("unsupported label count %d", e->M);
     return DSRG_E_INVALID;
diff --git a/dsrg_b200/csrc/srg.cu b/dsrg_b200/csrc/srg.cu
--- a/dsrg_b200/csrc/srg.cu
+++ b/dsrg_b200/csrc/srg.cu
@@ -1,4 +1,4 @@
-#include "common.cuh"
+#include "srg.cuh"
 
 namespace dsrg {
 
@@ -31,109 +31,50 @@
 #ifndef DSRG_SRG_LABEL_CTAS
 #define DSRG_SRG_LABEL_CTAS 1
 #endif
-template <bool CB>
-__device__ __forceinline__ float cue_at(const float *cues_f, const uint32_t *cues_b, size_t img_base_f, size_t img_base_w,
-                                        int c, int N, int i) {
-    if (!CB) return __ldg(cues_f + img_base_f + (size_t)c * N + i);
-    const size_t g = (size_t)c * N + i;
-    return (__ldg(cues_b + img_base_w + (g >> 5)) >> (g & 31)) & 1u ? 1.0f : 0.0f;
-}
-
-template <int MT, bool CB>
+template <int MT>
 __global__ void __launch_bounds__(kThreads, DSRG_SRG_LABEL_CTAS)
 k_srg_label(const float *__restrict__ labels, const float *__restrict__ probs, const float *__restrict__ cues,
-            const uint32_t *__restrict__ cue_bits, int wpi,
-            double th1, double th2, int renorm, uint8_t *lmap, uint8_t *lflag, int32_t *parent, uint8_t *hc,
-            int32_t *label_map_out, int Mrt, int N, int W) {
+            const uint32_t *__restrict__ cue_bits, int wpi, double th1, double th2, int renorm, uint8_t *lmap,
+            uint8_t *lflag, int32_t *parent, uint8_t *hc, int32_t *label_map_out, float *__restrict__ seeds, int Mrt,
+            int N, int W) {
     const int M = MT ? MT : Mrt;
     const int b = blockIdx.y;
     const int i = blockIdx.x * blockDim.x + threadIdx.x;
     const bool in = i < N;
     int L = 0;
     if (in) {
-        const float *lab = labels + (size_t)b * M;
         const float *pb = probs + (size_t)b * M * N + i;
         const size_t cbase_f = (size_t)b * M * N, cbase_w = (size_t)b * wpi;
-        int cstar = -1;
-        double best = 0.0, s = 0.0;
-        float nseed = 0.0f;
-        float cue_at_L = 0.0f;
         float cuv[MT ? MT : 1], pv[MT ? MT : 1];
         if (MT) {
 #pragma unroll
             for (int c = 0; c < (MT ? MT : 1); c++) {
-                cuv[c] = cue_at<CB>(cues, cue_bits, cbase_f, cbase_w, c, N, i);
+                cuv[c] = cue_at(cues, cue_bits, cbase_f, cbase_w, c, N, i);
                 pv[c] = __ldg(pb + (size_t)c * N);
             }
         }
-        constexpr bool kInline = MT >= 8 && MT <= 128;
-        constexpr int kBody = MT - MT % 8;
-        double r8[8] = {0, 0, 0, 0, 0, 0, 0, 0};
-#pragma unroll
-        for (int c = 0; c < M; c++) {
-            const float cu = MT ? cuv[MT ? c : 0] : cue_at<CB>(cues, cue_bits, cbase_f, cbase_w, c, N, i);
-            nseed += cu;
-            if (cu > 0.0f) {
-                L = c + 1;
-                cue_at_L = cu;
-            }
-            double v = (double)(MT ? pv[MT ? c : 0] : pb[(size_t)c * N]);
-            if (renorm && v < 0.0001) v = 0.0001;
-            if (kInline && renorm) {
-                if (c < 8) r8[c & 7] = v;
-                else if (c < kBody) r8[c & 7] += v;
-                else {
-                    if (c == kBody) s = ((r8[0] + r8[1]) + (r8[2] + r8[3])) + ((r8[4] + r8[5]) + (r8[6] + r8[7]));
-                    s += v;
-                }
-            }
-            if (lab[c] == 1.0f && (cstar < 0 || v > best)) {
-                best = v;
-                cstar = c;
-            }
-        }
-        if (renorm) {
-            if (kInline) {
-                if (MT == kBody) s = ((r8[0] + r8[1]) + (r8[2] + r8[3])) + ((r8[4] + r8[5]) + (r8[6] + r8[7]));
-            } else {
-                auto clamped = [&](int c) {
-                    const double v = (double)(MT ? pv[MT ? c : 0] : pb[(size_t)c * N]);
-                    return v < 0.0001 ? 0.0001 : v;
-                };
-                s = numpy_sum<MT>(clamped, M);
-            }
-            best = best / s;
-        }
-        if (cstar >= 0 && best > th2 && (cstar != 0 || best > th1)) {
-            L = cstar + 1;
-            cue_at_L = cue_at<CB>(cues, cue_bits, cbase_f, cbase_w, cstar, N, i);
-        }
-        uint8_t fl = 0;
-        if (L > 0) {
-            const bool present = lab[L - 1] == 1.0f;
-            const bool own = cue_at_L == 1.0f;
-            if (present && own) fl |= 1;
-            if (!own && nseed == 1.0f) fl |= 2;
-        }
+        auto prob = [&](int c) { return MT ? pv[MT ? c : 0] : pb[(size_t)c * N]; };
+        auto cue_mem = [&](int c) { return cue_at(cues, cue_bits, cbase_f, cbase_w, c, N, i); };
+        auto cue = [&](int c) {
+            const float cu = MT ? cuv[MT ? c : 0] : cue_mem(c);
+            if (seeds) seeds[cbase_f + (size_t)c * N + i] = cu;
+            return cu;
+        };
+        const float *lab = labels + (size_t)b * M;
+        int cstar;
+        const double best = srg_winner<MT>(prob, lab, M, renorm, cstar);
+        uint8_t fl;
+        L = srg_label<MT>(cue, cue_mem, lab, M, cstar, best, th1, th2, fl);
         lmap[(size_t)b * N + i] = (uint8_t)L;
         lflag[(size_t)b * N + i] = fl;
         hc[(size_t)b * N + i] = 0;
         if (label_map_out) label_map_out[(size_t)b * N + i] = L;
     }
-    const unsigned lane = threadIdx.x & 31;
-    const int x = in ? i % W : 0;
-    const int left = __shfl_up_sync(0xffffffffu, L, 1);
-    const bool joins_left = in && lane > 0 && x > 0 && L > 0 && left == L;
-    const unsigned brk = ~__ballot_sync(0xffffffffu, joins_left);
-    if (in) {
-        const unsigned below = brk & (0xffffffffu >> (31 - lane));
-        const int head_lane = 31 - __clz(below);
-        parent[(size_t)b * N + i] = i - ((int)lane - head_lane);
-    }
+    srg_link_runs(L, in, in ? i % W : 0, i, parent + (size_t)b * N);
 }
 
 __global__ void __launch_bounds__(kThreads)
-k_srg_merge(const uint8_t *lmap, int32_t *parent, int N, int W) {
+k_srg_merge(const uint8_t *lmap, int32_t *parent, int N, int W, int tile_w) {
     const int b = blockIdx.y;
     const int i = blockIdx.x * blockDim.x + threadIdx.x;
     if (i >= N) return;
@@ -142,7 +83,8 @@
     const int L = lm[i];
     if (L == 0) return;
     const int x = i % W;
-    if (x > 0 && (threadIdx.x & 31) == 0 && lm[i - 1] == L) uf_union(par, i, i - 1);
+    const bool win_start = tile_w ? x % tile_w == 0 : (i & 31) == 0;
+    if (x > 0 && win_start && lm[i - 1] == L) uf_union(par, i, i - 1);
     if (i >= W) {
         const int n = i - W;
         if (lm[n] == L) {
@@ -165,12 +107,10 @@
     if (lflag[(size_t)b * N + i] & 1) hc[(size_t)b * N + root] = 1;
 }
 
-template <int MT, bool CB, bool SB>
+template <bool SB>
 __global__ void __launch_bounds__(kThreads)
-k_srg_emit(const float *__restrict__ cues, const uint32_t *__restrict__ cue_bits, int wpi, const uint8_t *lmap,
-           const uint8_t *lflag, const int32_t *parent, const uint8_t *hc, float *__restrict__ seeds_out,
-           uint32_t *__restrict__ seed_bits, int Mrt, int N) {
-    const int M = MT ? MT : Mrt;
+k_srg_grow(const uint8_t *lmap, const uint8_t *lflag, const int32_t *parent, const uint8_t *hc,
+           float *__restrict__ seeds, uint32_t *__restrict__ seed_bits, int wpi, int M, int N) {
     const int b = blockIdx.y;
     const int i = blockIdx.x * blockDim.x + threadIdx.x;
     const bool in = i < N;
@@ -184,44 +124,37 @@
             if (hc[(size_t)b * N + root]) grow_c = L - 1;
         }
     }
-    const size_t cbase_f = (size_t)b * M * N, cbase_w = (size_t)b * wpi;
-    float *ob = seeds_out + (size_t)b * M * N + i;
-    const int i0 = i & ~31;
-    if (MT) {
-        float v[MT ? MT : 1];
-#pragma unroll
-        for (int c = 0; c < (MT ? MT : 1); c++) v[c] = in ? cue_at<CB>(cues, cue_bits, cbase_f, cbase_w, c, N, i) : 0.0f;
-#pragma unroll
-        for (int c = 0; c < (MT ? MT : 1); c++) {
-            const float o = (c == grow_c) ? 1.0f : v[c];
-            if (!SB) {
-                ob[(size_t)c * N] = o;
-            } else {
-                const unsigned m = __ballot_sync(0xffffffffu, in && o != 0.0f);
-                if ((threadIdx.x & 31) == 0 && m) {
-                    const size_t g0 = (size_t)c * N + i0;
-                    const int sh = (int)(g0 & 31);
-                    atomicOr(seed_bits + cbase_w + (g0 >> 5), m << sh);
-                    if (sh && (m >> (32 - sh))) atomicOr(seed_bits + cbase_w + (g0 >> 5) + 1, m >> (32 - sh));
-                }
-            }
-        }
-    } else {
-        for (int c = 0; c < M; c++) {
-            const float o = (c == grow_c) ? 1.0f : (in ? cue_at<CB>(cues, cue_bits, cbase_f, cbase_w, c, N, i) : 0.0f);
-            if (!SB) {
-                ob[(size_t)c * N] = o;
-            } else {
-                const unsigned m = __ballot_sync(0xffffffffu, in && o != 0.0f);
-                if ((threadIdx.x & 31) == 0 && m) {
-                    const size_t g0 = (size_t)c * N + i0;
-                    const int sh = (int)(g0 & 31);
-                    atomicOr(seed_bits + cbase_w + (g0 >> 5), m << sh);
-                    if (sh && (m >> (32 - sh))) atomicOr(seed_bits + cbase_w + (g0 >> 5) + 1, m >> (32 - sh));
-                }
-            }
-        }
+    if (!SB) {
+        if (grow_c >= 0) seeds[((size_t)b * M + grow_c) * N + i] = 1.0f;
+        return;
     }
+    const unsigned growing = __ballot_sync(0xffffffffu, grow_c >= 0);
+    if (grow_c < 0) return;
+    const unsigned m = __match_any_sync(growing, grow_c);
+    if ((int)(threadIdx.x & 31) != __ffs(m) - 1) return;
+    const size_t g0 = (size_t)grow_c * N + (i & ~31);
+    const int sh = (int)(g0 & 31);
+    uint32_t *wb = seed_bits + (size_t)b * wpi + (g0 >> 5);
+    atomicOr(wb, m << sh);
+    if (sh && (m >> (32 - sh))) atomicOr(wb + 1, m >> (32 - sh));
+}
+
+int srg_finish(Engine *e, int B, const SrgArgs &a, int tile_w, cudaStream_t s) {
+    const int N = e->N;
+    dim3 g(cdiv(N, kThreads), B);
+    if (a.seed_bits && a.seed_bits != a.cue_bits)
+        DSRG_CUDA_TRY(cudaMemcpyAsync(a.seed_bits, a.cue_bits, (size_t)B * a.wpi * sizeof(uint32_t),
+                                      cudaMemcpyDeviceToDevice, s));
+    DSRG_LAUNCH(e, T_SRG_MERGE, s, k_srg_merge<<<g, kThreads, 0, s>>>(e->lmap, e->parent, N, e->W, tile_w));
+    DSRG_LAUNCH(e, T_SRG_FLAG, s, k_srg_flag<<<g, kThreads, 0, s>>>(e->lflag, e->parent, e->hc, N));
+    if (a.seed_bits)
+        DSRG_LAUNCH(e, T_SRG_EMIT, s, (k_srg_grow<true><<<g, kThreads, 0, s>>>(e->lmap, e->lflag, e->parent, e->hc,
+                                                                               nullptr, a.seed_bits, a.wpi, e->M, N)));
+    else
+        DSRG_LAUNCH(e, T_SRG_EMIT, s, (k_srg_grow<false><<<g, kThreads, 0, s>>>(e->lmap, e->lflag, e->parent, e->hc,
+                                                                                a.seeds, nullptr, a.wpi, e->M, N)));
+    DSRG_CUDA_TRY(cudaGetLastError());
+    return DSRG_OK;
 }
 
 int srg_run(Engine *e, int B, const float *labels, const float *probs, const float *cues,
@@ -232,31 +165,16 @@
         set_error("SRG seed bits need cue bits");
         return DSRG_E_INVALID;
     }
-    const int wpi = (int)(((size_t)M * N + 31) / 32);
+    const SrgArgs a = srg_args(e, labels, cues, cue_bits, seeds_out, seed_bits, th1, th2);
     dim3 g(cdiv(N, kThreads), B);
-#define DSRG_LABEL(MTV, CBV)                                                                                          \
+#define DSRG_LABEL(MTV)                                                                                               \
     DSRG_LAUNCH(e, T_SRG_LABEL, s,                                                                                     \
-                (k_srg_label<MTV, CBV><<<g, kThreads, 0, s>>>(labels, probs, cues, cue_bits, wpi, th1, th2, renorm, e->lmap, \
-                                                              e->lflag, e->parent, e->hc, label_map_out, M, N, e->W)))
-    if (M == 21) { if (cue_bits) DSRG_LABEL(21, true); else DSRG_LABEL(21, false); }
-    else { if (cue_bits) DSRG_LABEL(0, true); else DSRG_LABEL(0, false); }
+                (k_srg_label<MTV><<<g, kThreads, 0, s>>>(labels, probs, cues, cue_bits, a.wpi, th1, th2, renorm, e->lmap, \
+                                                         e->lflag, e->parent, e->hc, label_map_out, a.seed_copy(), M, N, e->W)))
+    if (M == 21) DSRG_LABEL(21);
+    else DSRG_LABEL(0);
 #undef DSRG_LABEL
-    DSRG_LAUNCH(e, T_SRG_MERGE, s, k_srg_merge<<<g, kThreads, 0, s>>>(e->lmap, e->parent, N, e->W));
-    DSRG_LAUNCH(e, T_SRG_FLAG, s, k_srg_flag<<<g, kThreads, 0, s>>>(e->lflag, e->parent, e->hc, N));
-    if (seed_bits) DSRG_CUDA_TRY(cudaMemsetAsync(seed_bits, 0, (size_t)B * wpi * sizeof(uint32_t), s));
-#define DSRG_EMIT(MTV, CBV, SBV)                                                                                       \
-    DSRG_LAUNCH(e, T_SRG_EMIT, s,                                                                                      \
-                (k_srg_emit<MTV, CBV, SBV><<<g, kThreads, 0, s>>>(cues, cue_bits, wpi, e->lmap, e->lflag, e->parent, e->hc, \
-                                                                  seeds_out, seed_bits, M, N)))
-#define DSRG_EMIT_MT(MTV)                                              \
-    if (cue_bits && seed_bits) DSRG_EMIT(MTV, true, true);             \
-    else if (cue_bits) DSRG_EMIT(MTV, true, false);                    \
-    else DSRG_EMIT(MTV, false, false)
-    if (M == 21) { DSRG_EMIT_MT(21); } else { DSRG_EMIT_MT(0); }
-#undef DSRG_EMIT_MT
-#undef DSRG_EMIT
-    DSRG_CUDA_TRY(cudaGetLastError());
-    return DSRG_OK;
+    return srg_finish(e, B, a, 0, s);
 }
 
 }
diff --git a/dsrg_b200/csrc/srg.cuh b/dsrg_b200/csrc/srg.cuh
--- /dev/null
+++ b/dsrg_b200/csrc/srg.cuh
@@ -0,0 +1,118 @@
+#pragma once
+#include "common.cuh"
+
+namespace dsrg {
+
+struct SrgArgs {
+    const float *labels;
+    const float *cues;
+    const uint32_t *cue_bits;
+    float *seeds;
+    uint32_t *seed_bits;
+    int wpi;
+    double th1, th2;
+    uint8_t *lmap, *lflag, *hc;
+    int32_t *parent;
+    __host__ __device__ float *seed_copy() const { return seeds != cues ? seeds : nullptr; }
+};
+
+inline SrgArgs srg_args(const Engine *e, const float *labels, const float *cues, const uint32_t *cue_bits,
+                        float *seeds_out, uint32_t *seed_bits, double th1, double th2) {
+    const int wpi = (int)(((size_t)e->M * e->N + 31) / 32);
+    return SrgArgs{labels, cues, cue_bits, seed_bits ? nullptr : seeds_out, seed_bits, wpi, th1, th2,
+                   e->lmap, e->lflag, e->hc, e->parent};
+}
+
+__device__ __forceinline__ float cue_at(const float *cues_f, const uint32_t *cues_b, size_t img_base_f,
+                                        size_t img_base_w, int c, int N, int i) {
+    if (!cues_b) return __ldg(cues_f + img_base_f + (size_t)c * N + i);
+    const size_t g = (size_t)c * N + i;
+    return (__ldg(cues_b + img_base_w + (g >> 5)) >> (g & 31)) & 1u ? 1.0f : 0.0f;
+}
+
+template <int UT, typename P>
+__device__ __forceinline__ double srg_winner(P prob, const float *lab, int M, int renorm, int &cstar) {
+    static_assert(UT <= 128, "one NumPy summation block");
+    cstar = -1;
+    double best = 0.0, s = 0.0;
+    const int body = M - M % 8;
+    double r8[8] = {0, 0, 0, 0, 0, 0, 0, 0};
+#pragma unroll
+    for (int c = 0; c < (UT ? UT : M); c++) {
+        if (UT && c >= M) break;
+        double v = (double)prob(c);
+        if (renorm && v < 0.0001) v = 0.0001;
+        if (UT && renorm) {
+            if (c < body) {
+                if (c < 8) r8[c & 7] = v;
+                else r8[c & 7] += v;
+            } else {
+                if (c == body) s = ((r8[0] + r8[1]) + (r8[2] + r8[3])) + ((r8[4] + r8[5]) + (r8[6] + r8[7]));
+                s += v;
+            }
+        }
+        if (lab[c] == 1.0f && (cstar < 0 || v > best)) {
+            best = v;
+            cstar = c;
+        }
+    }
+    if (renorm) {
+        if (UT) {
+            if (M == body) s = ((r8[0] + r8[1]) + (r8[2] + r8[3])) + ((r8[4] + r8[5]) + (r8[6] + r8[7]));
+        } else {
+            auto clamped = [&](int c) {
+                const double v = (double)prob(c);
+                return v < 0.0001 ? 0.0001 : v;
+            };
+            s = numpy_sum<0>(clamped, M);
+        }
+        best = best / s;
+    }
+    return best;
+}
+
+template <int UT, typename C, typename CM>
+__device__ __forceinline__ int srg_label(C cue, CM cue_mem, const float *lab, int M, int cstar, double best,
+                                         double th1, double th2, uint8_t &fl) {
+    int L = 0;
+    float nseed = 0.0f;
+    float cue_at_L = 0.0f;
+#pragma unroll
+    for (int c = 0; c < (UT ? UT : M); c++) {
+        if (UT && c >= M) break;
+        const float cu = cue(c);
+        nseed += cu;
+        if (cu > 0.0f) {
+            L = c + 1;
+            cue_at_L = cu;
+        }
+    }
+    if (cstar >= 0 && best > th2 && (cstar != 0 || best > th1)) {
+        L = cstar + 1;
+        cue_at_L = cue_mem(cstar);
+    }
+    fl = 0;
+    if (L > 0) {
+        const bool present = lab[L - 1] == 1.0f;
+        const bool own = cue_at_L == 1.0f;
+        if (present && own) fl |= 1;
+        if (!own && nseed == 1.0f) fl |= 2;
+    }
+    return L;
+}
+
+__device__ __forceinline__ void srg_link_runs(int L, bool in, int x, int pix, int32_t *parent_img) {
+    const unsigned lane = threadIdx.x & 31;
+    const int left = __shfl_up_sync(0xffffffffu, L, 1);
+    const bool joins_left = in && lane > 0 && x > 0 && L > 0 && left == L;
+    const unsigned brk = ~__ballot_sync(0xffffffffu, joins_left);
+    if (in) {
+        const unsigned below = brk & (0xffffffffu >> (31 - lane));
+        const int head_lane = 31 - __clz(below);
+        parent_img[pix] = pix - ((int)lane - head_lane);
+    }
+}
+
+int srg_finish(Engine *e, int B, const SrgArgs &a, int tile_w, cudaStream_t s);
+
+}
```

After: 3486 (median of 6 runs). +1.5%, better.
